# slp-rl/slamkit

Measured on NVIDIA H100. Metric: speech-tokens/sec (SLAM seq=1024), higher is better.
Workload: dtype bf16

## Files before the change

slamkit_b200/csrc/common.cuh:

```cuda
#pragma once
#include <cuda_runtime.h>
#include <cuda_bf16.h>
#include <cuda.h>
#include <stdint.h>
#include <stdio.h>

#define SK_DEVINL __device__ __forceinline__

typedef __nv_bfloat16 bf16;
typedef __nv_bfloat162 bf162;

void sk_set_error(const char* fmt, ...);
#define SK_CUDA_CHECK(expr)                                                            \
  do {                                                                                 \
    cudaError_t _e = (expr);                                                           \
    if (_e != cudaSuccess) {                                                           \
      sk_set_error("%s:%d: %s -> %s", __FILE__, __LINE__, #expr, cudaGetErrorString(_e)); \
      return -2;                                                                       \
    }                                                                                  \
  } while (0)
void sk_count_launch();
#define SK_LAUNCH_CHECK()            \
  do {                               \
    sk_count_launch();               \
    SK_CUDA_CHECK(cudaGetLastError()); \
  } while (0)
#define SK_REQUIRE(cond, ...)                  \
  do {                                         \
    if (!(cond)) {                             \
      sk_set_error(__VA_ARGS__);               \
      return -1;                               \
    }                                          \
  } while (0)

int sk_num_sms();

#ifdef __CUDACC__
__device__ __forceinline__ void griddep_wait() { asm volatile("griddepcontrol.wait;" ::: "memory"); }
__device__ __forceinline__ void griddep_launch() { asm volatile("griddepcontrol.launch_dependents;" ::: "memory"); }
#endif
bool sk_pdl_enabled();
template <typename... KArgs, typename... Args>
inline cudaError_t sk_launch_pdl_if(bool pdl, void (*kernel)(KArgs...), dim3 grid, dim3 block, size_t smem, cudaStream_t s,
                                    Args... args) {
  cudaLaunchConfig_t cfg = {};
  cfg.gridDim = grid;
  cfg.blockDim = block;
  cfg.dynamicSmemBytes = smem;
  cfg.stream = s;
  cudaLaunchAttribute attr[1];
  attr[0].id = cudaLaunchAttributeProgrammaticStreamSerialization;
  attr[0].val.programmaticStreamSerializationAllowed = 1;
  cfg.attrs = attr;
  cfg.numAttrs = (pdl && sk_pdl_enabled()) ? 1 : 0;
  return cudaLaunchKernelEx(&cfg, kernel, static_cast<KArgs>(args)...);
}
template <typename... KArgs, typename... Args>
inline cudaError_t sk_launch_pdl(void (*kernel)(KArgs...), dim3 grid, dim3 block, size_t smem, cudaStream_t s, Args... args) {
  return sk_launch_pdl_if(true, kernel, grid, block, smem, s, args...);
}
void sk_prof_begin(int cat, cudaStream_t s);
void sk_prof_end(cudaStream_t s);

SK_DEVINL uint32_t pack_bf16(float lo, float hi) {
  bf162 v = __floats2bfloat162_rn(lo, hi);
  return *reinterpret_cast<uint32_t*>(&v);
}
SK_DEVINL float2 unpack_bf16(uint32_t v) {
  bf162 b = *reinterpret_cast<bf162*>(&v);
  return __bfloat1622float2(b);
}
SK_DEVINL float bf16_round(float x) { return __bfloat162float(__float2bfloat16_rn(x)); }

SK_DEVINL float warp_sum(float v) {
#pragma unroll
  for (int o = 16; o > 0; o >>= 1) v += __shfl_xor_sync(0xffffffffu, v, o);
  return v;
}
SK_DEVINL float warp_max(float v) {
#pragma unroll
  for (int o = 16; o > 0; o >>= 1) v = fmaxf(v, __shfl_xor_sync(0xffffffffu, v, o));
  return v;
}

SK_DEVINL uint4 ldg128(const void* p) { return __ldg(reinterpret_cast<const uint4*>(p)); }
SK_DEVINL uint4 ldg128_stream(const void* p) {
  uint4 r;
  asm volatile("ld.global.nc.L1::no_allocate.v4.u32 {%0,%1,%2,%3}, [%4];"
               : "=r"(r.x), "=r"(r.y), "=r"(r.z), "=r"(r.w)
               : "l"(p));
  return r;
}
SK_DEVINL void stg128(void* p, uint4 v) { *reinterpret_cast<uint4*>(p) = v; }

SK_DEVINL uint32_t smem_u32(const void* p) { return static_cast<uint32_t>(__cvta_generic_to_shared(p)); }

SK_DEVINL uint32_t elect_one() {
  uint32_t pred = 0;
  asm volatile(
      "{\n\t.reg .pred P;\n\t"
      "elect.sync _|P, 0xffffffff;\n\t"
      "selp.u32 %0, 1, 0, P;\n\t}\n"
      : "=r"(pred));
  return pred;
}

SK_DEVINL void mbar_init(uint32_t bar, uint32_t count) {
  asm volatile("mbarrier.init.shared::cta.b64 [%0], %1;" ::"r"(bar), "r"(count) : "memory");
}
SK_DEVINL void fence_mbar_init() { asm volatile("fence.mbarrier_init.release.cluster;" ::: "memory"); }
SK_DEVINL void fence_proxy_async() { asm volatile("fence.proxy.async.shared::cta;" ::: "memory"); }
SK_DEVINL void mbar_arrive(uint32_t bar) {
  asm volatile("mbarrier.arrive.shared::cta.b64 _, [%0];" ::"r"(bar) : "memory");
}
SK_DEVINL void mbar_arrive_expect_tx(uint32_t bar, uint32_t bytes) {
  asm volatile("mbarrier.arrive.expect_tx.shared::cta.b64 _, [%0], %1;" ::"r"(bar), "r"(bytes) : "memory");
}
SK_DEVINL uint32_t mbar_try_wait(uint32_t bar, uint32_t parity) {
  uint32_t ok;
  asm volatile(
      "{\n\t.reg .pred P;\n\t"
      "mbarrier.try_wait.parity.shared::cta.b64 P, [%1], %2;\n\t"
      "selp.u32 %0, 1, 0, P;\n\t}\n"
      : "=r"(ok)
      : "r"(bar), "r"(parity)
      : "memory");
  return ok;
}
SK_DEVINL uint64_t globaltimer_ns() {
  uint64_t t;
  asm volatile("mov.u64 %0, %%globaltimer;" : "=l"(t));
  return t;
}
SK_DEVINL float ex2_approx(float x) {
  float y;
  asm("ex2.approx.ftz.f32 %0, %1;" : "=f"(y) : "f"(x));
  return y;
}

SK_DEVINL float sigmoid_f(float x) {
  float r;
  asm("rcp.approx.ftz.f32 %0, %1;" : "=f"(r) : "f"(1.0f + ex2_approx(x * -1.4426950408889634f)));
  return r;
}
SK_DEVINL float silu_f(float x) { return x * sigmoid_f(x); }

typedef float2 f32x2;
SK_DEVINL f32x2 pk2(float a, float b) { return make_float2(a, b); }
SK_DEVINL void upk2(f32x2 v, float& a, float& b) { a = v.x; b = v.y; }
SK_DEVINL f32x2 dup2(float c) { return make_float2(c, c); }
SK_DEVINL f32x2 fma2(f32x2 a, f32x2 b, f32x2 c) { return make_float2(__fmaf_rn(a.x, b.x, c.x), __fmaf_rn(a.y, b.y, c.y)); }
SK_DEVINL f32x2 mul2(f32x2 a, f32x2 b) { return make_float2(__fmul_rn(a.x, b.x), __fmul_rn(a.y, b.y)); }
SK_DEVINL f32x2 add2(f32x2 a, f32x2 b) { return make_float2(__fadd_rn(a.x, b.x), __fadd_rn(a.y, b.y)); }
SK_DEVINL f32x2 sub2(f32x2 a, f32x2 b) { return make_float2(__fsub_rn(a.x, b.x), __fsub_rn(a.y, b.y)); }
SK_DEVINL void mbar_wait_sleep(uint32_t bar, uint32_t parity) {
  if (mbar_try_wait(bar, parity)) return;
  uint64_t t0 = globaltimer_ns();
  uint32_t spins = 0;
  while (!mbar_try_wait(bar, parity)) {
    __nanosleep(40);
    if ((++spins & 0xfffu) == 0 && globaltimer_ns() - t0 > 4000000000ull) {
      printf("slamkit_b200: mbarrier wait timeout (block %d thread %d bar 0x%x parity %u)\n", blockIdx.x, threadIdx.x, bar,
             parity);
      __trap();
    }
  }
}
SK_DEVINL void mbar_wait(uint32_t bar, uint32_t parity) {
  if (mbar_try_wait(bar, parity)) return;
  uint64_t t0 = globaltimer_ns();
  uint32_t spins = 0;
  while (!mbar_try_wait(bar, parity)) {
    if ((++spins & 0x3fffu) == 0) {
      if (globaltimer_ns() - t0 > 4000000000ull) {
        printf("slamkit_b200: mbarrier wait timeout (block %d thread %d bar 0x%x parity %u)\n", blockIdx.x,
               threadIdx.x, bar, parity);
        __trap();
      }
    }
  }
}

SK_DEVINL void mbar_wait_nocall(uint32_t bar, uint32_t parity) {
  if (mbar_try_wait(bar, parity)) return;
  uint64_t t0 = globaltimer_ns();
  uint32_t spins = 0;
  while (!mbar_try_wait(bar, parity)) {
    if ((++spins & 0x3fffu) == 0 && globaltimer_ns() - t0 > 4000000000ull) __trap();
  }
}

SK_DEVINL void tma_prefetch_desc(const void* tmap) {
  asm volatile("prefetch.tensormap [%0];" ::"l"(tmap) : "memory");
}
SK_DEVINL void tma_load_2d(uint32_t smem_dst, const void* tmap, uint32_t bar, int32_t c0, int32_t c1) {
  asm volatile(
      "cp.async.bulk.tensor.2d.shared::cluster.global.mbarrier::complete_tx::bytes [%0], [%1, {%3, %4}], [%2];"
      ::"r"(smem_dst), "l"(tmap), "r"(bar), "r"(c0), "r"(c1)
      : "memory");
}
SK_DEVINL void tma_load_3d(uint32_t smem_dst, const void* tmap, uint32_t bar, int32_t c0, int32_t c1, int32_t c2) {
  asm volatile(
      "cp.async.bulk.tensor.3d.shared::cluster.global.mbarrier::complete_tx::bytes [%0], [%1, {%3, %4, %5}], [%2];"
      ::"r"(smem_dst), "l"(tmap), "r"(bar), "r"(c0), "r"(c1), "r"(c2)
      : "memory");
}
SK_DEVINL void tma_store_2d(const void* tmap, uint32_t smem_src, int32_t c0, int32_t c1) {
  asm volatile("cp.async.bulk.tensor.2d.global.shared::cta.bulk_group [%0, {%2, %3}], [%1];" ::"l"(tmap),
               "r"(smem_src), "r"(c0), "r"(c1)
               : "memory");
}
SK_DEVINL void tma_store_commit() { asm volatile("cp.async.bulk.commit_group;" ::: "memory"); }
template <int N>
SK_DEVINL void tma_store_wait_read() {
  asm volatile("cp.async.bulk.wait_group.read %0;" ::"n"(N) : "memory");
}
template <int N>
SK_DEVINL void tma_store_wait() {
  asm volatile("cp.async.bulk.wait_group %0;" ::"n"(N) : "memory");
}

SK_DEVINL void wgmma_fence() { asm volatile("wgmma.fence.sync.aligned;" ::: "memory"); }
SK_DEVINL void wgmma_commit() { asm volatile("wgmma.commit_group.sync.aligned;" ::: "memory"); }
template <int N>
SK_DEVINL void wgmma_wait() {
  asm volatile("wgmma.wait_group.sync.aligned %0;" ::"n"(N) : "memory");
}
SK_DEVINL void named_bar_sync(int id, int threads) { asm volatile("bar.sync %0, %1;" ::"r"(id), "r"(threads) : "memory"); }

SK_DEVINL uint64_t gmma_desc_sw128(uint32_t smem_addr, uint32_t lbo_bytes, uint32_t sbo_bytes) {
  uint64_t d = 0;
  d |= (uint64_t)((smem_addr & 0x3ffffu) >> 4);
  d |= (uint64_t)((lbo_bytes >> 4) & 0x3fffu) << 16;
  d |= (uint64_t)((sbo_bytes >> 4) & 0x3fffu) << 32;
  d |= (uint64_t)1 << 62;
  return d;
}
template <int TA, int TB>
SK_DEVINL void wgmma_m64n64(float (&d)[32], uint64_t da, uint64_t db) {
  asm volatile(
      "{\n\t.reg .pred p;\n\tsetp.eq.u32 p, 1, 1;\n\t"
      "wgmma.mma_async.sync.aligned.m64n64k16.f32.bf16.bf16 {%0,%1,%2,%3,%4,%5,%6,%7,%8,%9,%10,%11,%12,%13,%14,%15,%16,%17,%18,%19,%20,%21,%22,%23,%24,%25,%26,%27,%28,%29,%30,%31}, %32, %33, p, 1, 1, %34, %35;\n\t}\n"
      : "+f"(d[0]), "+f"(d[1]), "+f"(d[2]), "+f"(d[3]), "+f"(d[4]), "+f"(d[5]), "+f"(d[6]), "+f"(d[7]), "+f"(d[8]), "+f"(d[9]), "+f"(d[10]), "+f"(d[11]), "+f"(d[12]), "+f"(d[13]), "+f"(d[14]), "+f"(d[15]), "+f"(d[16]), "+f"(d[17]), "+f"(d[18]), "+f"(d[19]), "+f"(d[20]), "+f"(d[21]), "+f"(d[22]), "+f"(d[23]), "+f"(d[24]), "+f"(d[25]), "+f"(d[26]), "+f"(d[27]), "+f"(d[28]), "+f"(d[29]), "+f"(d[30]), "+f"(d[31])
      : "l"(da), "l"(db), "n"(TA), "n"(TB));
}
template <int TA, int TB>
SK_DEVINL void wgmma_m64n128(float (&d)[64], uint64_t da, uint64_t db) {
  asm volatile(
      "{\n\t.reg .pred p;\n\tsetp.eq.u32 p, 1, 1;\n\t"
      "wgmma.mma_async.sync.aligned.m64n128k16.f32.bf16.bf16 {%0,%1,%2,%3,%4,%5,%6,%7,%8,%9,%10,%11,%12,%13,%14,%15,%16,%17,%18,%19,%20,%21,%22,%23,%24,%25,%26,%27,%28,%29,%30,%31,%32,%33,%34,%35,%36,%37,%38,%39,%40,%41,%42,%43,%44,%45,%46,%47,%48,%49,%50,%51,%52,%53,%54,%55,%56,%57,%58,%59,%60,%61,%62,%63}, %64, %65, p, 1, 1, %66, %67;\n\t}\n"
      : "+f"(d[0]), "+f"(d[1]), "+f"(d[2]), "+f"(d[3]), "+f"(d[4]), "+f"(d[5]), "+f"(d[6]), "+f"(d[7]), "+f"(d[8]), "+f"(d[9]), "+f"(d[10]), "+f"(d[11]), "+f"(d[12]), "+f"(d[13]), "+f"(d[14]), "+f"(d[15]), "+f"(d[16]), "+f"(d[17]), "+f"(d[18]), "+f"(d[19]), "+f"(d[20]), "+f"(d[21]), "+f"(d[22]), "+f"(d[23]), "+f"(d[24]), "+f"(d[25]), "+f"(d[26]), "+f"(d[27]), "+f"(d[28]), "+f"(d[29]), "+f"(d[30]), "+f"(d[31]), "+f"(d[32]), "+f"(d[33]), "+f"(d[34]), "+f"(d[35]), "+f"(d[36]), "+f"(d[37]), "+f"(d[38]), "+f"(d[39]), "+f"(d[40]), "+f"(d[41]), "+f"(d[42]), "+f"(d[43]), "+f"(d[44]), "+f"(d[45]), "+f"(d[46]), "+f"(d[47]), "+f"(d[48]), "+f"(d[49]), "+f"(d[50]), "+f"(d[51]), "+f"(d[52]), "+f"(d[53]), "+f"(d[54]), "+f"(d[55]), "+f"(d[56]), "+f"(d[57]), "+f"(d[58]), "+f"(d[59]), "+f"(d[60]), "+f"(d[61]), "+f"(d[62]), "+f"(d[63])
      : "l"(da), "l"(db), "n"(TA), "n"(TB));
}
template <int TA, int TB>
SK_DEVINL void wgmma_m64n256(float (&d)[128], uint64_t da, uint64_t db) {
  asm volatile(
      "{\n\t.reg .pred p;\n\tsetp.eq.u32 p, 1, 1;\n\t"
      "wgmma.mma_async.sync.aligned.m64n256k16.f32.bf16.bf16 {%0,%1,%2,%3,%4,%5,%6,%7,%8,%9,%10,%11,%12,%13,%14,%15,%16,%17,%18,%19,%20,%21,%22,%23,%24,%25,%26,%27,%28,%29,%30,%31,%32,%33,%34,%35,%36,%37,%38,%39,%40,%41,%42,%43,%44,%45,%46,%47,%48,%49,%50,%51,%52,%53,%54,%55,%56,%57,%58,%59,%60,%61,%62,%63,%64,%65,%66,%67,%68,%69,%70,%71,%72,%73,%74,%75,%76,%77,%78,%79,%80,%81,%82,%83,%84,%85,%86,%87,%88,%89,%90,%91,%92,%93,%94,%95,%96,%97,%98,%99,%100,%101,%102,%103,%104,%105,%106,%107,%108,%109,%110,%111,%112,%113,%114,%115,%116,%117,%118,%119,%120,%121,%122,%123,%124,%125,%126,%127}, %128, %129, p, 1, 1, %130, %131;\n\t}\n"
      : "+f"(d[0]), "+f"(d[1]), "+f"(d[2]), "+f"(d[3]), "+f"(d[4]), "+f"(d[5]), "+f"(d[6]), "+f"(d[7]), "+f"(d[8]), "+f"(d[9]), "+f"(d[10]), "+f"(d[11]), "+f"(d[12]), "+f"(d[13]), "+f"(d[14]), "+f"(d[15]), "+f"(d[16]), "+f"(d[17]), "+f"(d[18]), "+f"(d[19]), "+f"(d[20]), "+f"(d[21]), "+f"(d[22]), "+f"(d[23]), "+f"(d[24]), "+f"(d[25]), "+f"(d[26]), "+f"(d[27]), "+f"(d[28]), "+f"(d[29]), "+f"(d[30]), "+f"(d[31]), "+f"(d[32]), "+f"(d[33]), "+f"(d[34]), "+f"(d[35]), "+f"(d[36]), "+f"(d[37]), "+f"(d[38]), "+f"(d[39]), "+f"(d[40]), "+f"(d[41]), "+f"(d[42]), "+f"(d[43]), "+f"(d[44]), "+f"(d[45]), "+f"(d[46]), "+f"(d[47]), "+f"(d[48]), "+f"(d[49]), "+f"(d[50]), "+f"(d[51]), "+f"(d[52]), "+f"(d[53]), "+f"(d[54]), "+f"(d[55]), "+f"(d[56]), "+f"(d[57]), "+f"(d[58]), "+f"(d[59]), "+f"(d[60]), "+f"(d[61]), "+f"(d[62]), "+f"(d[63]), "+f"(d[64]), "+f"(d[65]), "+f"(d[66]), "+f"(d[67]), "+f"(d[68]), "+f"(d[69]), "+f"(d[70]), "+f"(d[71]), "+f"(d[72]), "+f"(d[73]), "+f"(d[74]), "+f"(d[75]), "+f"(d[76]), "+f"(d[77]), "+f"(d[78]), "+f"(d[79]), "+f"(d[80]), "+f"(d[81]), "+f"(d[82]), "+f"(d[83]), "+f"(d[84]), "+f"(d[85]), "+f"(d[86]), "+f"(d[87]), "+f"(d[88]), "+f"(d[89]), "+f"(d[90]), "+f"(d[91]), "+f"(d[92]), "+f"(d[93]), "+f"(d[94]), "+f"(d[95]), "+f"(d[96]), "+f"(d[97]), "+f"(d[98]), "+f"(d[99]), "+f"(d[100]), "+f"(d[101]), "+f"(d[102]), "+f"(d[103]), "+f"(d[104]), "+f"(d[105]), "+f"(d[106]), "+f"(d[107]), "+f"(d[108]), "+f"(d[109]), "+f"(d[110]), "+f"(d[111]), "+f"(d[112]), "+f"(d[113]), "+f"(d[114]), "+f"(d[115]), "+f"(d[116]), "+f"(d[117]), "+f"(d[118]), "+f"(d[119]), "+f"(d[120]), "+f"(d[121]), "+f"(d[122]), "+f"(d[123]), "+f"(d[124]), "+f"(d[125]), "+f"(d[126]), "+f"(d[127])
      : "l"(da), "l"(db), "n"(TA), "n"(TB));
}
template <int N, int TA, int TB>
SK_DEVINL void wgmma_bf16(float (&d)[N / 2], uint64_t da, uint64_t db) {
  if constexpr (N == 256) wgmma_m64n256<TA, TB>(d, da, db);
  else if constexpr (N == 128) wgmma_m64n128<TA, TB>(d, da, db);
  else wgmma_m64n64<TA, TB>(d, da, db);
}
```

slamkit_b200/csrc/gemm_tcgen05.cu:

```cuda
#include "common.cuh"
#include <cudaTypedefs.h>
#include <stdio.h>
#include <mutex>
#include <string.h>
#include <stdlib.h>
#include "kernels.h"
#include "../../include/slamkit_b200.h"

namespace {

constexpr int BM = 128;
constexpr int BK = 64;
constexpr int MMA_K = 16;
constexpr int GEMM_THREADS = 288;


struct GemmParams {
  int M, N, K;
  int batch;
  int a_mode;
  int passes;
  void* C;
  void* C_lo;
  int ldc;
  const void* bias;
  int bias_f32;
  const bf16* residual;
  const bf16* residual_lo;
  int ldr;
  int tiles_m, tiles_n;
  int out_f32;
  int round_before_res;
  int act;
  int col_gin, col_gout;
  int splits;
  float* splitk_ws;
  int tma_store;
  int pdl;
  int sk_units;
  int sk_groups;
  int sk_G;
  int sk_colunits;
  int units, n_groups;
  float* sk_ws;
  uint32_t* sk_flags;
  int epi;
  const bf16* aux;
  int ld_aux;
  const bf16* rope_cos;
  const bf16* rope_sin;
  const int* rope_pos;
  int rope_T, rope_cols, rope_maxpos;
};

template <int BN, int EW = 4>
struct GemmCfg {
  static constexpr int A_BYTES = BM * BK * 2;
  static constexpr int B_ATOMS = (BN + 63) / 64;
  static constexpr int B_BYTES = B_ATOMS * 64 * BK * 2;
  static constexpr int STAGE_BYTES = A_BYTES + B_BYTES;
  static constexpr int STAGES = (BN > 128) ? 4 : (BN > 64 ? 6 : 8);
  static constexpr int STAGING_BYTES = 4 * 2 * 4096;
  static constexpr int BAR_BYTES = 256;
  static constexpr int SMEM_BYTES = STAGES * STAGE_BYTES + STAGING_BYTES + BAR_BYTES + 1024;
  static_assert(STAGES * STAGE_BYTES >= BM * BN * 4, "the parked fp32 accumulator must fit in the stage ring");
  static_assert(SMEM_BYTES <= 227 * 1024, "sm_90 allows 227 KB of shared memory per block");
};

template <int BN>
SK_DEVINL uint32_t acc_chunk_addr(uint32_t base, int row, int chunk) {
  return base + (uint32_t)row * (BN * 4) + (uint32_t)((chunk ^ (row & 7)) << 4);
}
template <int BN>
SK_DEVINL void acc_park(uint32_t base, const float (&d)[BN / 2], int wg, int warp_in_wg, int lane) {
  const int r0 = 64 * wg + 16 * warp_in_wg + (lane >> 2);
#pragma unroll
  for (int j = 0; j < BN / 8; ++j) {
    const int chunk = 2 * j + ((lane & 3) >> 1);
    const uint32_t off = (uint32_t)(lane & 1) * 8u;
    asm volatile("st.shared.v2.f32 [%0], {%1, %2};" ::"r"(acc_chunk_addr<BN>(base, r0, chunk) + off), "f"(d[4 * j]),
                 "f"(d[4 * j + 1]) : "memory");
    asm volatile("st.shared.v2.f32 [%0], {%1, %2};" ::"r"(acc_chunk_addr<BN>(base, r0 + 8, chunk) + off), "f"(d[4 * j + 2]),
                 "f"(d[4 * j + 3]) : "memory");
  }
}
template <int BN>
SK_DEVINL void acc_ld_32x32(uint32_t base, uint32_t ta, uint32_t (&r)[32]) {
  const int row = (int)(ta >> 16) + (int)(threadIdx.x & 31);
  const int c0 = (int)(ta & 0xffffu) >> 2;
#pragma unroll
  for (int i = 0; i < 8; ++i)
    asm volatile("ld.shared.v4.b32 {%0, %1, %2, %3}, [%4];"
                 : "=r"(r[4 * i]), "=r"(r[4 * i + 1]), "=r"(r[4 * i + 2]), "=r"(r[4 * i + 3])
                 : "r"(acc_chunk_addr<BN>(base, row, c0 + i)) : "memory");
}

SK_DEVINL float gelu_erf(float y) {
  const float a = fabsf(y);
  float t;
  asm("rcp.approx.ftz.f32 %0, %1;" : "=f"(t) : "f"(fmaf(0.3275911f * 0.70710678118654752440f, a, 1.0f)));
  float s = fmaf(0.5f * 1.061405429f, t, 0.5f * -1.453152027f);
  s = fmaf(s, t, 0.5f * 1.421413741f);
  s = fmaf(s, t, 0.5f * -0.284496736f);
  s = fmaf(s, t, 0.5f * 0.254829592f);
  const float e = ex2_approx((y * y) * -0.72134752044448170368f);
  return fmaf(-a, (s * t) * e, fmaxf(y, 0.0f));
}

template <bool SK>
struct WorkIter {
  int num_kb, splits, kb_per_split, total_items, tiles_n;
  int G, colunits, units, n_groups, sk_groups, grp, mem;
  long sk_total, sk_cur, sk_end;
  int next_unit, next_item;
  int tile, split, kb_begin, kb_end, role;
  long unit_end_it;
  SK_DEVINL WorkIter(const GemmParams& p, int num_kb_, int kb_per_split_, int total_items_) {
    num_kb = num_kb_;
    splits = p.splits;
    kb_per_split = kb_per_split_;
    total_items = total_items_;
    tiles_n = p.tiles_n;
    G = p.sk_G;
    colunits = p.sk_colunits;
    units = p.units;
    n_groups = p.n_groups;
    sk_groups = p.sk_groups;
    tile = split = kb_begin = kb_end = role = 0;
    unit_end_it = 0;
    sk_total = sk_cur = sk_end = 0;
    next_item = (int)blockIdx.x;
    next_unit = 0;
    grp = mem = 0;
    if (SK && p.sk_units > 0) {
      grp = (int)blockIdx.x / G;
      mem = (int)blockIdx.x - grp * G;
      next_item = total_items;
      next_unit = grp < n_groups ? p.sk_units + grp : units;
      if (grp < sk_groups) {
        sk_total = (long)p.sk_units * num_kb;
        sk_cur = sk_total * grp / sk_groups;
        sk_end = sk_total * (grp + 1) / sk_groups;
      }
    }
  }
  SK_DEVINL int tile_of(int unit) const { return colunits ? mem * tiles_n + unit : unit * G + mem; }
  SK_DEVINL bool next() {
    if (SK && sk_cur < sk_end) {
      const int unit = (int)(sk_cur / num_kb);
      kb_begin = (int)(sk_cur - (long)unit * num_kb);
      unit_end_it = (long)(unit + 1) * num_kb;
      const long e = sk_end < unit_end_it ? sk_end : unit_end_it;
      kb_end = kb_begin + (int)(e - sk_cur);
      tile = tile_of(unit);
      split = 0;
      role = kb_begin != 0 ? 1 : (e < unit_end_it ? 2 : 0);
      sk_cur = e;
      return true;
    }
    if (SK && next_unit < units) {
      tile = tile_of(next_unit);
      split = 0;
      kb_begin = 0;
      kb_end = num_kb;
      role = 0;
      next_unit += n_groups;
      return true;
    }
    if (next_item < total_items) {
      split = next_item % splits;
      tile = next_item / splits;
      kb_begin = split * kb_per_split;
      kb_end = min(num_kb, kb_begin + kb_per_split);
      role = 0;
      next_item += (int)gridDim.x;
      return true;
    }
    return false;
  }
  SK_DEVINL int n_contrib() const {
    int n = 0;
    for (int g = grp + 1; g < sk_groups && sk_total * g / sk_groups < unit_end_it; ++g) ++n;
    return n;
  }
};

SK_DEVINL uint32_t ld_acquire_u32(const uint32_t* p) {
  uint32_t v;
  asm volatile("ld.acquire.gpu.global.u32 %0, [%1];" : "=r"(v) : "l"(p) : "memory");
  return v;
}
SK_DEVINL void st_release_u32(uint32_t* p, uint32_t v) {
  asm volatile("st.release.gpu.global.u32 [%0], %1;" ::"l"(p), "r"(v) : "memory");
}

SK_DEVINL void epi_bias_act(float (&v)[8], const GemmParams& p, int col) {
  if (p.bias) {
    if (p.bias_f32) {
      const float* bp = reinterpret_cast<const float*>(p.bias) + col;
      const float4 b0 = __ldg(reinterpret_cast<const float4*>(bp));
      const float4 b1 = __ldg(reinterpret_cast<const float4*>(bp + 4));
      v[0] += b0.x; v[1] += b0.y; v[2] += b0.z; v[3] += b0.w;
      v[4] += b1.x; v[5] += b1.y; v[6] += b1.z; v[7] += b1.w;
    } else {
      const uint4 bv = ldg128(reinterpret_cast<const bf16*>(p.bias) + col);
      const uint32_t bw[4] = {bv.x, bv.y, bv.z, bv.w};
#pragma unroll
      for (int i = 0; i < 4; ++i) {
        const float2 f = unpack_bf16(bw[i]);
        v[2 * i] += f.x;
        v[2 * i + 1] += f.y;
      }
    }
  }
  if (p.act == 1) {
#pragma unroll
    for (int i = 0; i < 8; ++i) v[i] = gelu_erf(v[i]);
  } else if (p.act == 2) {
#pragma unroll
    for (int i = 0; i < 8; ++i) v[i] = fmaxf(v[i], 0.0f);
  }
}

SK_DEVINL void epi_residual(float (&v)[8], const GemmParams& p, size_t row, int ocol) {
  if (!p.residual) return;
  const uint4 rv = *reinterpret_cast<const uint4*>(p.residual + row * p.ldr + ocol);
  const uint32_t rw[4] = {rv.x, rv.y, rv.z, rv.w};
#pragma unroll
  for (int i = 0; i < 4; ++i) {
    const float2 f = unpack_bf16(rw[i]);
    if (p.round_before_res) {
      v[2 * i] = bf16_round(v[2 * i]) + f.x;
      v[2 * i + 1] = bf16_round(v[2 * i + 1]) + f.y;
    } else {
      v[2 * i] += f.x;
      v[2 * i + 1] += f.y;
    }
  }
  if (p.residual_lo) {
    const uint4 lv = *reinterpret_cast<const uint4*>(p.residual_lo + row * p.ldr + ocol);
    const uint32_t lw[4] = {lv.x, lv.y, lv.z, lv.w};
#pragma unroll
    for (int i = 0; i < 4; ++i) {
      const float2 f = unpack_bf16(lw[i]);
      v[2 * i] += f.x;
      v[2 * i + 1] += f.y;
    }
  }
}

constexpr int SK_SLOT_FLOATS = BM * 256;
SK_DEVINL size_t sk_slot_off(int chunk, int j4, int row_in_tile) { return ((size_t)(chunk * 8 + j4) * BM + row_in_tile) * 4; }

SK_DEVINL void sk_fixup_add(uint32_t (&r)[32], const float* ws, int chunk, int row_in_tile, int first_cta, int G, int n) {
  for (int c0 = 0; c0 < n; ++c0) {
    const float* slot = ws + (size_t)(first_cta + c0 * G) * SK_SLOT_FLOATS;
    float4 a[8];
#pragma unroll
    for (int j = 0; j < 8; ++j) a[j] = __ldcg(reinterpret_cast<const float4*>(slot + sk_slot_off(chunk, j, row_in_tile)));
#pragma unroll
    for (int j = 0; j < 8; ++j) {
      r[4 * j + 0] = __float_as_uint(__uint_as_float(r[4 * j + 0]) + a[j].x);
      r[4 * j + 1] = __float_as_uint(__uint_as_float(r[4 * j + 1]) + a[j].y);
      r[4 * j + 2] = __float_as_uint(__uint_as_float(r[4 * j + 2]) + a[j].z);
      r[4 * j + 3] = __float_as_uint(__uint_as_float(r[4 * j + 3]) + a[j].w);
    }
  }
}

template <int BN, bool A_MN, bool B_MN, bool SK, int EW>
__global__ void __launch_bounds__(GEMM_THREADS, 1)
gemm_wgmma_kernel(const __grid_constant__ CUtensorMap tmA, const __grid_constant__ CUtensorMap tmB,
                  const __grid_constant__ CUtensorMap tmA_lo, const __grid_constant__ CUtensorMap tmB_lo,
                  const __grid_constant__ CUtensorMap tmC, const __grid_constant__ CUtensorMap tmAux, GemmParams p) {
  using Cfg = GemmCfg<BN, EW>;
  static_assert(EW == 4 || (EW == 8 && BN == 256 && !SK), "8 epilogue warps: plain 256-wide tiles only");
  constexpr int CS = EW / 4;
  griddep_launch();
  extern __shared__ uint8_t smem_raw[];
  const uint32_t smem_base = (smem_u32(smem_raw) + 1023u) & ~1023u;
  const uint32_t staging_base = smem_base + Cfg::STAGES * Cfg::STAGE_BYTES;
  const uint32_t bar_base = staging_base + Cfg::STAGING_BYTES;
  auto full_bar = [&](int s) { return bar_base + 8u * s; };
  auto empty_bar = [&](int s) { return bar_base + 8u * (Cfg::STAGES + s); };
  const uint32_t acc_free = bar_base + 8u * (2 * Cfg::STAGES);

  const int warp = threadIdx.x >> 5;
  const int lane = threadIdx.x & 31;
  const int tiles_per_batch = p.tiles_m * p.tiles_n;
  const int total_items = tiles_per_batch * p.batch * p.splits;
  const int num_kb_total = (p.K + BK - 1) / BK;
  const int kb_per_split = (num_kb_total + p.splits - 1) / p.splits;
  constexpr uint32_t STAGE_TX = Cfg::A_BYTES + (B_MN ? Cfg::B_ATOMS * 64 * BK * 2 : BN * BK * 2);

  if (threadIdx.x == 0) {
    tma_prefetch_desc(&tmA);
    tma_prefetch_desc(&tmB);
    for (int s = 0; s < Cfg::STAGES; ++s) {
      mbar_init(full_bar(s), 1);
      mbar_init(empty_bar(s), 8);
    }
    mbar_init(acc_free, 1);
    fence_mbar_init();
  }
  __syncthreads();
  griddep_wait();

  if (warp == 8) {
    if (lane == 0) {
      const bool split = p.passes == 3;
      const int n_stage = split ? Cfg::STAGES / 2 : Cfg::STAGES;
      const uint32_t stage_bytes = split ? 2u * Cfg::STAGE_BYTES : (uint32_t)Cfg::STAGE_BYTES;
      int stage = 0;
      uint32_t phase = 0;
      uint32_t acc_phase = 0;
      bool first = true;
      WorkIter<SK> w(p, num_kb_total, kb_per_split, total_items);
      while (w.next()) {
        if (!first) {
          mbar_wait_nocall(acc_free, acc_phase);
          acc_phase ^= 1u;
        }
        first = false;
        const int bidx = w.tile / tiles_per_batch;
        const int r = w.tile - bidx * tiles_per_batch;
        const int m0 = (r / p.tiles_n) * BM;
        const int n_blk = r % p.tiles_n;
        const int n0 = n_blk * BN;
        for (int kb = w.kb_begin; kb < w.kb_end; ++kb) {
          mbar_wait_nocall(empty_bar(stage), phase ^ 1u);
          const uint32_t fb = full_bar(stage);
          mbar_arrive_expect_tx(fb, split ? 2u * STAGE_TX : STAGE_TX);
          for (int part = 0; part < (split ? 2 : 1); ++part) {
            const CUtensorMap* mapA = part ? &tmA_lo : &tmA;
            const CUtensorMap* mapB = part ? &tmB_lo : &tmB;
            const uint32_t sA = smem_base + stage * stage_bytes + part * Cfg::STAGE_BYTES;
            const uint32_t sB = sA + Cfg::A_BYTES;
            if (!A_MN) {
              if (p.a_mode & 2) {
                if (p.a_mode & 1) tma_load_3d(sA, mapA, fb, n_blk * 64, m0 + kb, bidx);
                else tma_load_3d(sA, mapA, fb, kb * BK, m0, bidx);
              } else {
                tma_load_2d(sA, mapA, fb, kb * BK, m0);
              }
            } else {
#pragma unroll
              for (int j = 0; j < BM / 64; ++j) tma_load_2d(sA + j * (BK * 128), mapA, fb, m0 + 64 * j, kb * BK);
            }
            if (!B_MN) {
              tma_load_2d(sB, mapB, fb, kb * BK, n0);
            } else {
#pragma unroll
              for (int j = 0; j < Cfg::B_ATOMS; ++j) tma_load_2d(sB + j * (BK * 128), mapB, fb, n0 + 64 * j, kb * BK);
            }
          }
          if (++stage == n_stage) { stage = 0; phase ^= 1u; }
        }
      }
    }
  } else {
    const int wg = warp >> 2;
    const int q = warp & 3;
    const int chalf = warp >> 2;
    const bool epi_warp = warp < EW;
    auto acc_ld = [&](uint32_t ta, uint32_t (&r)[32]) { acc_ld_32x32<BN>(smem_base, ta, r); };
    const bool split = p.passes == 3;
    const int n_stage = split ? Cfg::STAGES / 2 : Cfg::STAGES;
    const uint32_t stage_bytes = split ? 2u * Cfg::STAGE_BYTES : (uint32_t)Cfg::STAGE_BYTES;
    int stage = 0;
    uint32_t phase = 0;
    uint32_t store_cnt = 0;
    auto release_acc = [&] {
      fence_proxy_async();
      named_bar_sync(1, 256);
      if (threadIdx.x == 0) mbar_arrive(acc_free);
    };
    WorkIter<SK> w(p, num_kb_total, kb_per_split, total_items);
    while (w.next()) {
      {
        float acc[BN / 2];
#pragma unroll
        for (int i = 0; i < BN / 2; ++i) acc[i] = 0.f;
        const int k_iters = max(0, w.kb_end - w.kb_begin);
        int prev = -1;
        for (int kb = 0; kb < k_iters; ++kb) {
          mbar_wait_nocall(full_bar(stage), phase);
          wgmma_fence();
          const uint32_t s_hi = smem_base + stage * stage_bytes;
          for (int g = 0; g < (split ? 3 : 1); ++g) {
            const uint32_t sA = s_hi + (g == 2 ? Cfg::STAGE_BYTES : 0) + (uint32_t)wg * 8192u;
            const uint32_t sB = s_hi + Cfg::A_BYTES + (g == 1 ? Cfg::STAGE_BYTES : 0);
#pragma unroll
            for (int k = 0; k < BK / MMA_K; ++k) {
              const uint64_t adesc = A_MN ? gmma_desc_sw128(sA + k * (MMA_K * 128), BK * 128, 1024)
                                          : gmma_desc_sw128(sA + k * (MMA_K * 2), 16, 1024);
              const uint64_t bdesc = B_MN ? gmma_desc_sw128(sB + k * (MMA_K * 128), BK * 128, 1024)
                                          : gmma_desc_sw128(sB + k * (MMA_K * 2), 16, 1024);
              wgmma_bf16<BN, A_MN ? 1 : 0, B_MN ? 1 : 0>(acc, adesc, bdesc);
            }
          }
          wgmma_commit();
          wgmma_wait<1>();
          if (prev >= 0 && lane == 0) mbar_arrive(empty_bar(prev));
          prev = stage;
          if (++stage == n_stage) { stage = 0; phase ^= 1u; }
        }
        wgmma_wait<0>();
        if (prev >= 0 && lane == 0) mbar_arrive(empty_bar(prev));
        named_bar_sync(1, 256);
        acc_park<BN>(smem_base, acc, wg, warp & 3, lane);
        named_bar_sync(1, 256);
      }
      if (!epi_warp) {
        release_acc();
        continue;
      }
      const int split_idx = w.split;
      const int bidx = w.tile / tiles_per_batch;
      const int rr = w.tile - bidx * tiles_per_batch;
      const int m0 = (rr / p.tiles_n) * BM;
      const int n0 = (rr % p.tiles_n) * BN;
      if (!SK && p.tma_store && p.epi == 2) {
        const int lpiece = lane & 7, lrsub = lane >> 3;
        const uint32_t sX = staging_base + (uint32_t)warp * (EW == 4 ? 8192u : 4096u);
        constexpr int NCH = BN / 64 / CS;
        const int c_lo = chalf * NCH;
        auto piece_off = [&](int bidx, int m0, int n0, int c2, size_t ld) -> size_t {
          const int acol = n0 + c2 * 64;
          const int gcol = (acol >> 7) * 256 + (acol & 127) + lpiece * 8;
          return (((size_t)bidx * p.M + m0 + q * 32 + lrsub) * ld + gcol) * sizeof(bf16);
        };
        const size_t row4_in = (size_t)4 * p.ld_aux * sizeof(bf16), row4_out = (size_t)4 * p.ldc * sizeof(bf16);
        uint4 gv[8], uv[8];
        auto gu_load_k = [&](int k, const uint8_t* base, int m0, int n0, int c2) {
          const int rin = m0 + q * 32 + 4 * k + lrsub;
          if (rin < p.M && n0 + c2 * 64 < p.N) {
            gv[k] = ldg128(base + k * row4_in);
            uv[k] = ldg128(base + k * row4_in + 256);
          } else {
            gv[k] = make_uint4(0u, 0u, 0u, 0u);
            uv[k] = make_uint4(0u, 0u, 0u, 0u);
          }
        };
        {
          const uint8_t* base = reinterpret_cast<const uint8_t*>(p.aux) + piece_off(bidx, m0, n0, c_lo, (size_t)p.ld_aux);
#pragma unroll
          for (int k = 0; k < 8; ++k) gu_load_k(k, base, m0, n0, c_lo);
        }
        const uint32_t taddr = (uint32_t)(q * 32) << 16;
#pragma unroll 1
        for (int c2 = c_lo; c2 < c_lo + NCH; ++c2) {
          const bool col_ok = n0 + c2 * 64 < p.N;
          {
            uint32_t r0[32], r1[32];
            acc_ld(taddr + c2 * 64, r0);
            acc_ld(taddr + c2 * 64 + 32, r1);
#pragma unroll
            for (int j = 0; j < 8; ++j) {
              const uint32_t* r = j < 4 ? r0 + 8 * j : r1 + 8 * (j - 4);
              const uint32_t dst = sX + (uint32_t)lane * 128u + (uint32_t)((j ^ (lane & 7)) << 4);
              asm volatile("st.shared.v4.b32 [%0], {%1, %2, %3, %4};" ::"r"(dst),
                           "r"(pack_bf16(__uint_as_float(r[0]), __uint_as_float(r[1]))),
                           "r"(pack_bf16(__uint_as_float(r[2]), __uint_as_float(r[3]))),
                           "r"(pack_bf16(__uint_as_float(r[4]), __uint_as_float(r[5]))),
                           "r"(pack_bf16(__uint_as_float(r[6]), __uint_as_float(r[7])))
                           : "memory");
            }
          }
          __syncwarp();
          const bool refill = c2 + 1 < c_lo + NCH;
          const int fm0 = m0, fn0 = n0, fc2 = c2 + 1;
          const uint8_t* fbase = reinterpret_cast<const uint8_t*>(p.aux) + piece_off(bidx, fm0, fn0, fc2, (size_t)p.ld_aux);
          uint8_t* obase = reinterpret_cast<uint8_t*>(p.C) + piece_off(bidx, m0, n0, c2, (size_t)p.ldc);
#pragma unroll
          for (int k = 0; k < 8; ++k) {
            const int rr2 = 4 * k + lrsub;
            const uint32_t off = (uint32_t)rr2 * 128u + (uint32_t)((lpiece ^ (rr2 & 7)) << 4);
            uint32_t dw[4];
            asm volatile("ld.shared.v4.b32 {%0, %1, %2, %3}, [%4];" : "=r"(dw[0]), "=r"(dw[1]), "=r"(dw[2]), "=r"(dw[3]) : "r"(sX + off));
            const uint32_t gw[4] = {gv[k].x, gv[k].y, gv[k].z, gv[k].w}, uw[4] = {uv[k].x, uv[k].y, uv[k].z, uv[k].w};
            if (refill) gu_load_k(k, fbase, fm0, fn0, fc2);
            uint32_t og[4], ou[4];
#pragma unroll
            for (int e = 0; e < 4; ++e) {
              const float2 gf = unpack_bf16(gw[e]);
              const float s0 = sigmoid_f(gf.x), s1 = sigmoid_f(gf.y);
              const uint32_t sil2 = pack_bf16(gf.x * s0, gf.y * s1);
              const float ds0 = s0 * (1.0f + gf.x * (1.0f - s0)), ds1 = s1 * (1.0f + gf.y * (1.0f - s1));
              const bf162 d2 = *reinterpret_cast<const bf162*>(&dw[e]);
              bf162 du2 = __hmul2(d2, *reinterpret_cast<const bf162*>(&uw[e]));
              bf162 o2 = __hmul2(d2, *reinterpret_cast<const bf162*>(&sil2));
              const float2 duf = __bfloat1622float2(du2);
              og[e] = pack_bf16(duf.x * ds0, duf.y * ds1);
              ou[e] = *reinterpret_cast<uint32_t*>(&o2);
            }
            if (col_ok && m0 + q * 32 + rr2 < p.M) {
              stg128(obase + k * row4_out, make_uint4(og[0], og[1], og[2], og[3]));
              stg128(obase + k * row4_out + 256, make_uint4(ou[0], ou[1], ou[2], ou[3]));
            }
          }
          __syncwarp();
        }
        release_acc();
        continue;
      }
      const int row_in_tile = q * 32 + lane;
      const int row_in = m0 + row_in_tile;
      const bool row_ok = row_in < p.M;
      const size_t row = (size_t)bidx * p.M + row_in;
      const uint32_t taddr = (uint32_t)(q * 32) << 16;
      const int first_contrib = (int)blockIdx.x + w.G;
      const int n_contrib = (SK && w.role == 2) ? w.n_contrib() : 0;
      if (SK && w.role == 1) {
        float* slot = p.sk_ws + (size_t)blockIdx.x * SK_SLOT_FLOATS;
#pragma unroll 1
        for (int c = 0; c < BN / 32; ++c) {
          uint32_t r[32];
          acc_ld(taddr + c * 32, r);
#pragma unroll
          for (int j = 0; j < 8; ++j)
            __stcg(reinterpret_cast<float4*>(slot + sk_slot_off(c, j, row_in_tile)),
                   make_float4(__uint_as_float(r[4 * j]), __uint_as_float(r[4 * j + 1]), __uint_as_float(r[4 * j + 2]),
                               __uint_as_float(r[4 * j + 3])));
        }
        __threadfence();
        __syncwarp();
        if (lane == 0) st_release_u32(p.sk_flags + blockIdx.x * 4 + q, 1u);
      } else {
        if (SK && w.role == 2) {
          if (lane == 0) {
            for (int i = 0; i < n_contrib; ++i) {
              const int c = first_contrib + i * w.G;
              const uint32_t* f = p.sk_flags + c * 4 + q;
              const uint64_t t0 = globaltimer_ns();
              while (ld_acquire_u32(f) == 0u) {
                __nanosleep(64);
                if (globaltimer_ns() - t0 > 8000000000ull) __trap();
              }
            }
          }
          __syncwarp();
        }
        auto stage_store = [&](const CUtensorMap* map, const uint32_t (&pk)[32], int col) {
          const uint32_t sbuf = staging_base + (EW == 4 ? (uint32_t)warp * 8192u + (store_cnt & 1u) * 4096u : (uint32_t)warp * 4096u);
          if (lane == 0) {
            if constexpr (EW == 4) tma_store_wait_read<1>(); else tma_store_wait_read<0>();
          }
          __syncwarp();
#pragma unroll
          for (int j = 0; j < 8; ++j) {
            const uint32_t dst = sbuf + (uint32_t)lane * 128u + (uint32_t)((j ^ (lane & 7)) << 4);
            asm volatile("st.shared.v4.b32 [%0], {%1, %2, %3, %4};" ::"r"(dst), "r"(pk[4 * j]), "r"(pk[4 * j + 1]),
                         "r"(pk[4 * j + 2]), "r"(pk[4 * j + 3])
                         : "memory");
          }
          fence_proxy_async();
          __syncwarp();
          if (lane == 0) {
            tma_store_2d(map, sbuf, col, m0 + q * 32);
            tma_store_commit();
          }
          ++store_cnt;
        };
        if (!SK && p.tma_store && p.epi == 1) {
          if constexpr (BN == 256) {
#pragma unroll 1
#pragma unroll 1
            for (int i = chalf * (2 / CS); i < (chalf + 1) * (2 / CS); ++i) {
              uint32_t gpk[32], upk[32];
              {
                uint32_t r0[32], r1[32];
                acc_ld(taddr + i * 64, r0);
                acc_ld(taddr + i * 64 + 32, r1);
#pragma unroll
                for (int t = 0; t < 16; ++t) {
                  gpk[t] = pack_bf16(__uint_as_float(r0[2 * t]), __uint_as_float(r0[2 * t + 1]));
                  gpk[16 + t] = pack_bf16(__uint_as_float(r1[2 * t]), __uint_as_float(r1[2 * t + 1]));
                }
              }
              stage_store(&tmC, gpk, n0 + i * 64);
              {
                uint32_t r0[32], r1[32];
                acc_ld(taddr + 128 + i * 64, r0);
                acc_ld(taddr + 128 + i * 64 + 32, r1);
#pragma unroll
                for (int t = 0; t < 16; ++t) {
                  upk[t] = pack_bf16(__uint_as_float(r0[2 * t]), __uint_as_float(r0[2 * t + 1]));
                  upk[16 + t] = pack_bf16(__uint_as_float(r1[2 * t]), __uint_as_float(r1[2 * t + 1]));
                }
              }
              stage_store(&tmC, upk, n0 + 128 + i * 64);
#pragma unroll
              for (int t = 0; t < 32; ++t) {
                const float2 gf = unpack_bf16(gpk[t]), uf = unpack_bf16(upk[t]);
                const float2 sb = unpack_bf16(pack_bf16(silu_f(gf.x), silu_f(gf.y)));
                gpk[t] = pack_bf16(sb.x * uf.x, sb.y * uf.y);
              }
              stage_store(&tmAux, gpk, (n0 >> 1) + i * 64);
            }
          }
        } else if (!SK && p.tma_store && p.epi == 3) {
          uint32_t cw[16], sw[16];
          {
            int pos = 0;
            if (row_ok) pos = p.rope_pos ? p.rope_pos[row] : (int)(row % (size_t)p.rope_T);
            pos = max(0, min(pos, p.rope_maxpos - 1));
#pragma unroll
            for (int j = 0; j < 4; ++j) {
              const uint4 c = ldg128(p.rope_cos + (size_t)pos * 32 + 8 * j), sn = ldg128(p.rope_sin + (size_t)pos * 32 + 8 * j);
              cw[4 * j] = c.x; cw[4 * j + 1] = c.y; cw[4 * j + 2] = c.z; cw[4 * j + 3] = c.w;
              sw[4 * j] = sn.x; sw[4 * j + 1] = sn.y; sw[4 * j + 2] = sn.z; sw[4 * j + 3] = sn.w;
            }
          }
#pragma unroll 1
          for (int c2 = chalf * (BN / 64 / CS); c2 < (chalf + 1) * (BN / 64 / CS); ++c2) {
            const int col64 = n0 + c2 * 64;
            if (col64 >= p.N) break;
            uint32_t r0[32], r1[32], pk[32];
            acc_ld(taddr + c2 * 64, r0);
            acc_ld(taddr + c2 * 64 + 32, r1);
#pragma unroll
            for (int g = 0; g < 4; ++g) {
              float v0[8], v1[8];
#pragma unroll
              for (int i = 0; i < 8; ++i) {
                v0[i] = __uint_as_float(r0[g * 8 + i]);
                v1[i] = __uint_as_float(r1[g * 8 + i]);
              }
              if (p.bias) {
                const uint4 b0 = ldg128(reinterpret_cast<const bf16*>(p.bias) + col64 + g * 8);
                const uint4 b1 = ldg128(reinterpret_cast<const bf16*>(p.bias) + col64 + 32 + g * 8);
                const uint32_t w0[4] = {b0.x, b0.y, b0.z, b0.w}, w1[4] = {b1.x, b1.y, b1.z, b1.w};
#pragma unroll
                for (int e = 0; e < 4; ++e) {
                  const float2 f0 = unpack_bf16(w0[e]), f1 = unpack_bf16(w1[e]);
                  v0[2 * e] += f0.x; v0[2 * e + 1] += f0.y;
                  v1[2 * e] += f1.x; v1[2 * e + 1] += f1.y;
                }
              }
              if (col64 < p.rope_cols) {
#pragma unroll
                for (int e = 0; e < 4; ++e) {
                  const float2 c = unpack_bf16(cw[g * 4 + e]), sn = unpack_bf16(sw[g * 4 + e]);
                  const float2 x1 = unpack_bf16(pack_bf16(v0[2 * e], v0[2 * e + 1]));
                  const float2 x2 = unpack_bf16(pack_bf16(v1[2 * e], v1[2 * e + 1]));
                  v0[2 * e] = bf16_round(x1.x * c.x) + bf16_round(-x2.x * sn.x);
                  v0[2 * e + 1] = bf16_round(x1.y * c.y) + bf16_round(-x2.y * sn.y);
                  v1[2 * e] = bf16_round(x2.x * c.x) + bf16_round(x1.x * sn.x);
                  v1[2 * e + 1] = bf16_round(x2.y * c.y) + bf16_round(x1.y * sn.y);
                }
              }
#pragma unroll
              for (int e = 0; e < 4; ++e) {
                pk[g * 4 + e] = pack_bf16(v0[2 * e], v0[2 * e + 1]);
                pk[16 + g * 4 + e] = pack_bf16(v1[2 * e], v1[2 * e + 1]);
              }
            }
            stage_store(&tmC, pk, col64);
          }
        } else if (p.tma_store && !p.bias && !p.residual && !p.act) {
#pragma unroll 1
          for (int c2 = chalf * (BN / 64 / CS); c2 < (chalf + 1) * (BN / 64 / CS); ++c2) {
            uint32_t r0[32], r1[32], pk[32];
            acc_ld(taddr + c2 * 64, r0);
            acc_ld(taddr + c2 * 64 + 32, r1);
            if (SK && n_contrib > 0) {
              sk_fixup_add(r0, p.sk_ws, c2 * 2, row_in_tile, first_contrib, w.G, n_contrib);
              sk_fixup_add(r1, p.sk_ws, c2 * 2 + 1, row_in_tile, first_contrib, w.G, n_contrib);
            }
#pragma unroll
            for (int t = 0; t < 16; ++t) {
              pk[t] = pack_bf16(__uint_as_float(r0[2 * t]), __uint_as_float(r0[2 * t + 1]));
              pk[16 + t] = pack_bf16(__uint_as_float(r1[2 * t]), __uint_as_float(r1[2 * t + 1]));
            }
            stage_store(&tmC, pk, n0 + c2 * 64);
          }
        } else if (p.tma_store && !p.bias && !p.act && p.residual && !p.residual_lo) {
#pragma unroll 1
          for (int c2 = chalf * (BN / 64 / CS); c2 < (chalf + 1) * (BN / 64 / CS); ++c2) {
            const int col64 = n0 + c2 * 64;
            if (col64 >= p.N) break;
            uint4 rv[8];
            if (row_ok) {
              const bf16* rp = p.residual + row * p.ldr + col64;
#pragma unroll
              for (int j = 0; j < 8; ++j) rv[j] = (col64 + 8 * j < p.N) ? ldg128(rp + 8 * j) : make_uint4(0u, 0u, 0u, 0u);
            } else {
#pragma unroll
              for (int j = 0; j < 8; ++j) rv[j] = make_uint4(0u, 0u, 0u, 0u);
            }
            uint32_t r0[32], r1[32], pk[32];
            acc_ld(taddr + c2 * 64, r0);
            acc_ld(taddr + c2 * 64 + 32, r1);
            if (SK && n_contrib > 0) {
              sk_fixup_add(r0, p.sk_ws, c2 * 2, row_in_tile, first_contrib, w.G, n_contrib);
              sk_fixup_add(r1, p.sk_ws, c2 * 2 + 1, row_in_tile, first_contrib, w.G, n_contrib);
            }
#pragma unroll
            for (int j = 0; j < 8; ++j) {
              const uint32_t* r = j < 4 ? r0 + 8 * j : r1 + 8 * (j - 4);
              const uint32_t rw[4] = {rv[j].x, rv[j].y, rv[j].z, rv[j].w};
#pragma unroll
              for (int e = 0; e < 4; ++e) {
                const float2 f = unpack_bf16(rw[e]);
                float a0 = __uint_as_float(r[2 * e]), a1 = __uint_as_float(r[2 * e + 1]);
                if (p.round_before_res) {
                  const float2 t = unpack_bf16(pack_bf16(a0, a1));
                  a0 = t.x; a1 = t.y;
                }
                pk[4 * j + e] = pack_bf16(a0 + f.x, a1 + f.y);
              }
            }
            stage_store(&tmC, pk, col64);
          }
        } else if (p.tma_store) {
#pragma unroll 1
          for (int c2 = chalf * (BN / 64 / CS); c2 < (chalf + 1) * (BN / 64 / CS); ++c2) {
            const uint32_t sbuf = staging_base + (EW == 4 ? (uint32_t)warp * 8192u + (store_cnt & 1u) * 4096u : (uint32_t)warp * 4096u);
            if (lane == 0) {
              if constexpr (EW == 4) tma_store_wait_read<1>(); else tma_store_wait_read<0>();
            }
            __syncwarp();
#pragma unroll
            for (int half = 0; half < 2; ++half) {
              uint32_t r[32];
              acc_ld(taddr + c2 * 64 + half * 32, r);
              if (SK && n_contrib > 0) sk_fixup_add(r, p.sk_ws, c2 * 2 + half, row_in_tile, first_contrib, w.G, n_contrib);
#pragma unroll
              for (int g = 0; g < 4; ++g) {
                const int col = n0 + c2 * 64 + half * 32 + g * 8;
                float v[8];
#pragma unroll
                for (int i = 0; i < 8; ++i) v[i] = __uint_as_float(r[g * 8 + i]);
                if (col < p.N) {
                  epi_bias_act(v, p, col);
                  if (row_ok) epi_residual(v, p, row, col);
                }
                const int j = half * 4 + g;
                const uint32_t dst = sbuf + (uint32_t)lane * 128u + (uint32_t)((j ^ (lane & 7)) << 4);
                asm volatile("st.shared.v4.b32 [%0], {%1, %2, %3, %4};" ::"r"(dst), "r"(pack_bf16(v[0], v[1])),
                             "r"(pack_bf16(v[2], v[3])), "r"(pack_bf16(v[4], v[5])), "r"(pack_bf16(v[6], v[7]))
                             : "memory");
              }
            }
            fence_proxy_async();
            __syncwarp();
            if (lane == 0) {
              tma_store_2d(&tmC, sbuf, n0 + c2 * 64, m0 + q * 32);
              tma_store_commit();
            }
            ++store_cnt;
          }
        }
        else
#pragma unroll 1
        for (int c = chalf * (BN / 32 / CS); c < (chalf + 1) * (BN / 32 / CS); ++c) {
          uint32_t r[32];
          acc_ld(taddr + c * 32, r);
          if (SK && n_contrib > 0) sk_fixup_add(r, p.sk_ws, c, row_in_tile, first_contrib, w.G, n_contrib);
          const int col0 = n0 + c * 32;
          if (row_ok && col0 < p.N) {
#pragma unroll
            for (int g = 0; g < 4; ++g) {
              const int col = col0 + g * 8;
              if (col < p.N) {
                float v[8];
#pragma unroll
                for (int i = 0; i < 8; ++i) v[i] = __uint_as_float(r[g * 8 + i]);
                if (p.splits > 1) {
                  float* dst = p.splitk_ws + ((size_t)split_idx * p.M + row_in) * p.N + col;
                  *reinterpret_cast<float4*>(dst) = make_float4(v[0], v[1], v[2], v[3]);
                  *reinterpret_cast<float4*>(dst + 4) = make_float4(v[4], v[5], v[6], v[7]);
                  continue;
                }
                epi_bias_act(v, p, col);
                int ocol = col;
                if (p.col_gin > 0) {
                  const int gi = col / p.col_gin, ci = col - gi * p.col_gin;
                  if (ci >= p.col_gout) continue;
                  ocol = gi * p.col_gout + ci;
                }
                epi_residual(v, p, row, ocol);
                if (p.out_f32) {
                  float* dst = reinterpret_cast<float*>(p.C) + row * p.ldc + ocol;
                  *reinterpret_cast<float4*>(dst) = make_float4(v[0], v[1], v[2], v[3]);
                  *reinterpret_cast<float4*>(dst + 4) = make_float4(v[4], v[5], v[6], v[7]);
                } else {
                  uint4 o;
                  o.x = pack_bf16(v[0], v[1]);
                  o.y = pack_bf16(v[2], v[3]);
                  o.z = pack_bf16(v[4], v[5]);
                  o.w = pack_bf16(v[6], v[7]);
                  stg128(reinterpret_cast<bf16*>(p.C) + row * p.ldc + ocol, o);
                  if (p.C_lo) {
                    const float2 h0 = unpack_bf16(o.x), h1 = unpack_bf16(o.y), h2 = unpack_bf16(o.z), h3 = unpack_bf16(o.w);
                    uint4 l;
                    l.x = pack_bf16(v[0] - h0.x, v[1] - h0.y);
                    l.y = pack_bf16(v[2] - h1.x, v[3] - h1.y);
                    l.z = pack_bf16(v[4] - h2.x, v[5] - h2.y);
                    l.w = pack_bf16(v[6] - h3.x, v[7] - h3.y);
                    stg128(reinterpret_cast<bf16*>(p.C_lo) + row * p.ldc + ocol, l);
                  }
                }
              }
            }
          }
        }
        if (SK && w.role == 2) {
          __syncwarp();
          if (lane == 0)
            for (int i = 0; i < n_contrib; ++i) p.sk_flags[(first_contrib + i * w.G) * 4 + q] = 0u;
        }
      }
      release_acc();
    }
    if (epi_warp && p.tma_store && lane == 0) tma_store_wait<0>();
  }
}

__global__ void splitk_reduce_kernel(const float* __restrict__ ws, bf16* __restrict__ C, int M, int N, int ldc, int splits,
                                     int accumulate, int round_before_res) {
  griddep_launch();
  griddep_wait();
  const long total = (long)M * N / 8;
  for (long i = blockIdx.x * (long)blockDim.x + threadIdx.x; i < total; i += (long)gridDim.x * blockDim.x) {
    const long e = i * 8;
    const int m = (int)(e / N), n = (int)(e % N);
    float acc[8] = {0, 0, 0, 0, 0, 0, 0, 0};
    for (int s = 0; s < splits; ++s) {
      const float* src = ws + ((size_t)s * M + m) * N + n;
      const float4 a = *reinterpret_cast<const float4*>(src), b = *reinterpret_cast<const float4*>(src + 4);
      acc[0] += a.x; acc[1] += a.y; acc[2] += a.z; acc[3] += a.w;
      acc[4] += b.x; acc[5] += b.y; acc[6] += b.z; acc[7] += b.w;
    }
    bf16* dst = C + (size_t)m * ldc + n;
    if (accumulate) {
      const uint4 o = *reinterpret_cast<const uint4*>(dst);
      const uint32_t ow[4] = {o.x, o.y, o.z, o.w};
#pragma unroll
      for (int k = 0; k < 4; ++k) {
        const float2 f = unpack_bf16(ow[k]);
        acc[2 * k] = (round_before_res ? bf16_round(acc[2 * k]) : acc[2 * k]) + f.x;
        acc[2 * k + 1] = (round_before_res ? bf16_round(acc[2 * k + 1]) : acc[2 * k + 1]) + f.y;
      }
    }
    stg128(dst, make_uint4(pack_bf16(acc[0], acc[1]), pack_bf16(acc[2], acc[3]), pack_bf16(acc[4], acc[5]),
                           pack_bf16(acc[6], acc[7])));
  }
}

PFN_cuTensorMapEncodeTiled_v12000 g_encode = nullptr;
std::once_flag g_encode_once;

void load_encode() {
  void* fn = nullptr;
  cudaDriverEntryPointQueryResult qres;
  cudaError_t e = cudaGetDriverEntryPoint("cuTensorMapEncodeTiled", &fn, cudaEnableDefault, &qres);
  if (e == cudaSuccess && qres == cudaDriverEntryPointSuccess) g_encode = (PFN_cuTensorMapEncodeTiled_v12000)fn;
}

}

int sk_make_tmap_2d(CUtensorMap* out, const void* ptr, int elem_bytes, uint64_t inner, uint64_t outer, uint64_t ld,
                    uint32_t box_inner, uint32_t box_outer) {
  std::call_once(g_encode_once, load_encode);
  SK_REQUIRE(g_encode != nullptr, "cuTensorMapEncodeTiled driver entry point not available");
  SK_REQUIRE((reinterpret_cast<uintptr_t>(ptr) & 15) == 0, "TMA base pointer must be 16-byte aligned");
  SK_REQUIRE((ld * elem_bytes) % 16 == 0, "TMA row pitch must be a multiple of 16 bytes (ld=%llu)",
             (unsigned long long)ld);
  SK_REQUIRE(box_inner * elem_bytes == 128, "SW128 box inner extent must be 128 bytes");
  cuuint64_t dims[2] = {inner, outer};
  cuuint64_t strides[1] = {ld * (uint64_t)elem_bytes};
  cuuint32_t box[2] = {box_inner, box_outer};
  cuuint32_t estr[2] = {1, 1};
  CUtensorMapDataType dt = elem_bytes == 2 ? CU_TENSOR_MAP_DATA_TYPE_BFLOAT16 : CU_TENSOR_MAP_DATA_TYPE_FLOAT32;
  CUresult r = g_encode(out, dt, 2, const_cast<void*>(ptr), dims, strides, box, estr, CU_TENSOR_MAP_INTERLEAVE_NONE,
                        CU_TENSOR_MAP_SWIZZLE_128B, CU_TENSOR_MAP_L2_PROMOTION_L2_256B,
                        CU_TENSOR_MAP_FLOAT_OOB_FILL_NONE);
  SK_REQUIRE(r == CUDA_SUCCESS, "cuTensorMapEncodeTiled failed with CUresult %d (inner=%llu outer=%llu ld=%llu)", (int)r,
             (unsigned long long)inner, (unsigned long long)outer, (unsigned long long)ld);
  return 0;
}

int sk_make_tmap_3d(CUtensorMap* out, const void* ptr, uint64_t inner, uint64_t rows, uint64_t batch, uint64_t row_stride,
                    uint64_t batch_stride, uint32_t box_rows) {
  std::call_once(g_encode_once, load_encode);
  SK_REQUIRE(g_encode != nullptr, "cuTensorMapEncodeTiled driver entry point not available");
  SK_REQUIRE((reinterpret_cast<uintptr_t>(ptr) & 15) == 0, "TMA base pointer must be 16-byte aligned");
  SK_REQUIRE((row_stride * 2) % 16 == 0 && (batch_stride * 2) % 16 == 0, "TMA strides must be multiples of 16 bytes");
  cuuint64_t dims[3] = {inner, rows, batch};
  cuuint64_t strides[2] = {row_stride * 2, batch_stride * 2};
  cuuint32_t box[3] = {64, box_rows, 1};
  cuuint32_t estr[3] = {1, 1, 1};
  CUresult r = g_encode(out, CU_TENSOR_MAP_DATA_TYPE_BFLOAT16, 3, const_cast<void*>(ptr), dims, strides, box, estr,
                        CU_TENSOR_MAP_INTERLEAVE_NONE, CU_TENSOR_MAP_SWIZZLE_128B, CU_TENSOR_MAP_L2_PROMOTION_L2_256B,
                        CU_TENSOR_MAP_FLOAT_OOB_FILL_NONE);
  SK_REQUIRE(r == CUDA_SUCCESS, "cuTensorMapEncodeTiled(3d) failed with CUresult %d", (int)r);
  return 0;
}

namespace {

template <int BN, bool A_MN, bool B_MN, bool SK, int EW = 4>
int launch_gemm(const CUtensorMap* tm, const GemmParams& p, int grid, cudaStream_t stream) {
  using Cfg = GemmCfg<BN, EW>;
  static bool attr_set = false;
  if (!attr_set) {
    SK_CUDA_CHECK(cudaFuncSetAttribute(gemm_wgmma_kernel<BN, A_MN, B_MN, SK, EW>, cudaFuncAttributeMaxDynamicSharedMemorySize,
                                       Cfg::SMEM_BYTES));
    attr_set = true;
  }
  sk_prof_begin(0, stream);
  cudaError_t lerr = sk_launch_pdl_if(p.pdl != 0, gemm_wgmma_kernel<BN, A_MN, B_MN, SK, EW>, dim3(grid), dim3(GEMM_THREADS), (size_t)Cfg::SMEM_BYTES, stream,
                                   tm[0], tm[1], tm[2], tm[3], tm[4], tm[5], p);
  sk_prof_end(stream);
  SK_CUDA_CHECK(lerr);
  SK_LAUNCH_CHECK();
  return 0;
}

template <int BN, bool SK, int EW = 4>
int dispatch_major(bool a_mn, bool b_mn, const CUtensorMap* tm, const GemmParams& p, int grid, cudaStream_t s) {
  if (!a_mn && !b_mn) return launch_gemm<BN, false, false, SK, EW>(tm, p, grid, s);
  if (!a_mn && b_mn) return launch_gemm<BN, false, true, SK, EW>(tm, p, grid, s);
  if (a_mn && !b_mn) return launch_gemm<BN, true, false, SK, EW>(tm, p, grid, s);
  return launch_gemm<BN, true, true, SK, EW>(tm, p, grid, s);
}

inline int tile_cost(int bn) { return bn >= 256 ? 100 : (bn >= 128 ? 61 : 54); }

constexpr size_t SK_FLAG_BYTES = 4096;

}

size_t sk_gemm_ws_min_bytes(void) { return (size_t)sk_num_sms() * SK_SLOT_FLOATS * sizeof(float) + SK_FLAG_BYTES; }

int sk_pick_bn(int M, int N, int force_bn) {
  if (force_bn == 64 || force_bn == 128 || force_bn == 256) return force_bn;
  const int nsm = sk_num_sms();
  const int cands[3] = {256, 128, 64};
  int best = 256;
  long best_cost = -1;
  for (int i = 0; i < 3; ++i) {
    const int bn = cands[i];
    const long tiles = (long)((M + BM - 1) / BM) * ((N + bn - 1) / bn);
    const long waves = (tiles + nsm - 1) / nsm;
    const long cost = waves * tile_cost(bn);
    if (best_cost < 0 || cost * 100 < best_cost * 75) {
      best_cost = cost;
      best = bn;
    }
  }
  return best;
}

namespace {

int plan_gemm(const SkGemmEx& g, GemmParams& p, int& BN, int& ew, int& grid) {
  SK_REQUIRE(g.M > 0 && g.N > 0 && g.K > 0 && g.batch >= 1, "gemm: empty problem M=%d N=%d K=%d batch=%d", g.M, g.N, g.K,
             g.batch);
  SK_REQUIRE(g.N % 8 == 0, "gemm: N must be a multiple of 8 (N=%d)", g.N);
  SK_REQUIRE(g.ldc % 8 == 0 && (g.residual == nullptr || g.ldr % 8 == 0), "gemm: ldc/ldr must be multiples of 8");
  SK_REQUIRE((reinterpret_cast<uintptr_t>(g.C) & 15) == 0, "gemm: C must be 16-byte aligned");
  SK_REQUIRE(((reinterpret_cast<uintptr_t>(g.A) | reinterpret_cast<uintptr_t>(g.B) | reinterpret_cast<uintptr_t>(g.A_lo) |
               reinterpret_cast<uintptr_t>(g.B_lo)) & 15) == 0,
             "gemm: A and B must be 16-byte aligned");
  SK_REQUIRE((reinterpret_cast<uintptr_t>(g.bias) & 15) == 0 && (reinterpret_cast<uintptr_t>(g.residual) & 15) == 0,
             "gemm: bias and residual must be 16-byte aligned");
  SK_REQUIRE(g.passes == 1 || (g.passes == 3 && g.A_lo && g.B_lo), "gemm: passes must be 1, or 3 with lo operands");
  SK_REQUIRE(g.act >= 0 && g.act <= 2, "gemm: act must be 0 (none), 1 (GELU) or 2 (ReLU), got %d", g.act);
  const bool use3d = g.a_rows > 0;
  SK_REQUIRE(!use3d || !g.a_mn, "gemm: a batched / windowed A operand must be K-major");
  SK_REQUIRE(g.a_mode == 0 || use3d, "gemm: a_mode 1 needs the 3-D A view");
  SK_REQUIRE(use3d || g.lda >= (g.a_mn ? g.M : g.K), "gemm: lda=%d is smaller than the %s of A", g.lda, g.a_mn ? "M" : "K");
  SK_REQUIRE(g.ldb >= (g.b_mn ? g.N : g.K), "gemm: ldb=%d is smaller than the %s of B", g.ldb, g.b_mn ? "N" : "K");
  if (g.col_gin == 0) {
    const int out_cols = g.epi == 2 ? 2 * g.N : g.N;
    SK_REQUIRE(g.ldc >= out_cols, "gemm: ldc=%d is smaller than the %d output columns", g.ldc, out_cols);
    SK_REQUIRE(g.residual == nullptr || g.ldr >= g.N, "gemm: ldr=%d is smaller than N=%d", g.ldr, g.N);
  }
  const int nsm = sk_num_sms();
  static const int sk_env = [] { const char* e = getenv("SK_STREAMK"); return e ? atoi(e) : 1; }();
  static const int sk_min_idle = [] { const char* e = getenv("SK_STREAMK_MIN_IDLE"); return e ? atoi(e) : 20; }();
  static const int sk_min_kb = [] { const char* e = getenv("SK_STREAMK_MIN_KB"); return e ? atoi(e) : 32; }();
  const bool sk_ok = sk_env != 0 && g.batch == 1 && !use3d && g.passes == 1 && g.a_mode == 0 && g.splitk_ws != nullptr &&
                     g.splitk_ws_bytes >= sk_gemm_ws_min_bytes();
  const size_t ws_data_bytes = g.splitk_ws_bytes > SK_FLAG_BYTES ? g.splitk_ws_bytes - SK_FLAG_BYTES : 0;
  BN = (g.a_mode == 1) ? 64 : sk_pick_bn(g.M * g.batch, g.N, (g.epi == 1 || g.epi == 2) ? 256 : g.force_bn);
  memset(&p, 0, sizeof(p));
  p.M = g.M; p.N = g.N; p.K = g.K;
  p.batch = g.batch;
  p.a_mode = (g.a_mode & 1) | (use3d ? 2 : 0);
  p.passes = g.passes;
  p.C = g.C; p.C_lo = g.C_lo; p.ldc = g.ldc;
  p.bias = g.bias; p.bias_f32 = g.bias_f32;
  p.residual = reinterpret_cast<const bf16*>(g.residual);
  p.residual_lo = reinterpret_cast<const bf16*>(g.residual_lo);
  p.ldr = g.ldr;
  p.tiles_m = (g.M + BM - 1) / BM;
  p.tiles_n = (g.N + BN - 1) / BN;
  p.out_f32 = g.out_f32;
  p.round_before_res = g.round_before_res;
  p.act = g.act;
  p.col_gin = g.col_gin; p.col_gout = g.col_gout;
  p.pdl = g.pdl;
  const long tiles = (long)p.tiles_m * p.tiles_n * g.batch;
  p.splits = 1;
  p.splitk_ws = nullptr;
  const int num_kb = (g.K + BK - 1) / BK;
  static const int splitk_env = [] { const char* e = getenv("SK_SPLITK"); return e ? atoi(e) : 1; }();
  static const int sk_ranges = [] { const char* e = getenv("SK_STREAMK_RANGES"); return e ? atoi(e) : 4; }();
  if (splitk_env && g.splitk_ws && g.batch == 1 && g.passes == 1 && !g.out_f32 && !g.bias && !g.act && !g.C_lo && g.col_gin == 0 &&
      (g.residual == nullptr || g.residual == g.C) && tiles * 2 <= nsm && num_kb >= 16) {
    int sp = (int)(nsm / tiles);
    if (sp > 8) sp = 8;
    if (sp > num_kb / 4) sp = num_kb / 4;
    if ((size_t)sp * g.M * g.N * sizeof(float) > ws_data_bytes) sp = (int)(ws_data_bytes / ((size_t)g.M * g.N * sizeof(float)));
    if (sp >= 2) {
      const int per = (num_kb + sp - 1) / sp;
      sp = (num_kb + per - 1) / per;
    }
    if (sp >= 2) {
      p.splits = sp;
      p.splitk_ws = reinterpret_cast<float*>(g.splitk_ws);
    }
  }
  p.tma_store = (!g.out_f32 && !g.C_lo && g.col_gin == 0 && p.splits == 1 && g.batch == 1 && !use3d && (g.ldc * 2) % 16 == 0)
                    ? 1 : 0;
  p.epi = g.epi;
  p.aux = reinterpret_cast<const bf16*>(g.aux);
  p.ld_aux = g.ld_aux;
  p.rope_cos = reinterpret_cast<const bf16*>(g.rope_cos);
  p.rope_sin = reinterpret_cast<const bf16*>(g.rope_sin);
  p.rope_pos = g.rope_pos;
  p.rope_T = g.rope_T; p.rope_cols = g.rope_cols; p.rope_maxpos = g.rope_maxpos;
  if (g.epi != 0) {
    SK_REQUIRE(p.tma_store && g.passes == 1 && !g.residual && !g.act && g.splitk_ws == nullptr,
               "gemm: fused epilogue %d needs the plain bf16 TMA-store path (no residual / activation / scratch)", g.epi);
    if (g.epi == 1) {
      SK_REQUIRE(BN == 256 && g.N % 256 == 0 && g.aux_out && g.ld_aux_out % 8 == 0 && !g.bias,
                 "gemm: SwiGLU-forward epilogue needs N = 2F with F %% 128 == 0 and an act output");
    } else if (g.epi == 2) {
      SK_REQUIRE(BN == 256 && g.N % 128 == 0 && g.aux && g.ld_aux % 8 == 0 && !g.bias,
                 "gemm: SwiGLU-backward epilogue needs N = F with F %% 128 == 0 and the saved gu activation");
    } else if (g.epi == 3) {
      SK_REQUIRE(g.rope_cos && g.rope_sin && g.rope_T > 0 && g.rope_maxpos > 0 && g.rope_cols % 64 == 0 && g.N % 64 == 0 &&
                     !g.bias_f32,
                 "gemm: RoPE epilogue needs cos/sin tables, 64-column heads and a bf16 bias");
    } else {
      SK_REQUIRE(false, "gemm: unknown fused epilogue %d", g.epi);
    }
  }
  p.sk_G = 1;
  if (sk_ok && BN == 256 && p.splits == 1 && num_kb >= sk_min_kb && (p.tiles_n <= 8 || (sk_env >= 2 && p.tiles_m <= 8))) {
    const int colunits = p.tiles_n <= 8 ? 0 : 1;
    const int G = colunits ? p.tiles_m : p.tiles_n;
    const int units = colunits ? p.tiles_n : p.tiles_m;
    const int n_groups = nsm / G;
    const int rem = units % n_groups;
    const long slots = ((long)(units + n_groups - 1) / n_groups) * n_groups;
    if (n_groups >= 1 && rem != 0 && (slots - units) * 100 >= slots * sk_min_idle) {
      p.sk_units = rem;
      p.sk_groups = n_groups < rem * sk_ranges ? n_groups : rem * sk_ranges;
      p.sk_G = G;
      p.sk_colunits = colunits;
      p.units = units;
      p.n_groups = n_groups;
      p.sk_ws = reinterpret_cast<float*>(g.splitk_ws);
      p.sk_flags = reinterpret_cast<uint32_t*>(reinterpret_cast<uint8_t*>(g.splitk_ws) + ws_data_bytes);
    }
  }
  const long work = tiles * p.splits;
  grid = p.sk_units > 0 ? p.n_groups * p.sk_G : (int)(work < nsm ? work : nsm);
  static const int ew_env = [] { const char* e = getenv("SK_GEMM_EW"); return e ? atoi(e) : 0; }();
  ew = (p.sk_units == 0 && BN == 256 && p.tma_store && (ew_env == 8 || (ew_env == 0 && (g.epi == 2 || g.epi == 3)))) ? 8 : 4;
  return 0;
}

}

int sk_gemm_plan_ex(const SkGemmEx& g, SkGemmPlan* out) {
  GemmParams p;
  int BN = 0, ew = 0, grid = 0;
  const int rc = plan_gemm(g, p, BN, ew, grid);
  if (rc) return rc;
  out->bn = BN;
  out->epi_warps = ew;
  out->splits = p.splits;
  out->sk_units = p.sk_units;
  out->sk_groups = p.sk_groups;
  out->sk_G = p.sk_G;
  out->sk_colunits = p.sk_colunits;
  out->tma_store = p.tma_store;
  out->grid = grid;
  return 0;
}

int sk_gemm_ex_launch(const SkGemmEx& g, cudaStream_t stream) {
  GemmParams p;
  int BN = 0, ew = 0, grid = 0;
  const int rc0 = plan_gemm(g, p, BN, ew, grid);
  if (rc0) return rc0;
  const bool use3d = g.a_rows > 0;
  CUtensorMap tm[6];
  const void* As[2] = {g.A, g.passes == 3 ? g.A_lo : g.A};
  const void* Bs[2] = {g.B, g.passes == 3 ? g.B_lo : g.B};
  for (int i = 0; i < 2; ++i) {
    int rc;
    CUtensorMap* ta = &tm[i == 0 ? 0 : 2];
    CUtensorMap* tb = &tm[i == 0 ? 1 : 3];
    if (use3d) {
      rc = sk_make_tmap_3d(ta, As[i], (uint64_t)g.a_inner, (uint64_t)g.a_rows, (uint64_t)g.batch, (uint64_t)g.a_row_stride,
                           (uint64_t)g.a_batch_stride, BM);
    } else if (!g.a_mn) {
      rc = sk_make_tmap_2d(ta, As[i], 2, (uint64_t)g.K, (uint64_t)g.M, (uint64_t)g.lda, BK, BM);
    } else {
      rc = sk_make_tmap_2d(ta, As[i], 2, (uint64_t)g.M, (uint64_t)g.K, (uint64_t)g.lda, 64, BK);
    }
    if (rc) return rc;
    if (!g.b_mn) rc = sk_make_tmap_2d(tb, Bs[i], 2, (uint64_t)g.K, (uint64_t)g.N, (uint64_t)g.ldb, BK, (uint32_t)BN);
    else         rc = sk_make_tmap_2d(tb, Bs[i], 2, (uint64_t)g.N, (uint64_t)g.K, (uint64_t)g.ldb, 64, BK);
    if (rc) return rc;
  }
  tm[4] = tm[0];
  if (p.tma_store) {
    const int rc2 = sk_make_tmap_2d(&tm[4], g.C, 2, (uint64_t)(g.epi == 2 ? 2 * g.N : g.N), (uint64_t)g.M, (uint64_t)g.ldc, 64, 32);
    if (rc2) return rc2;
  }
  tm[5] = tm[4];
  if (g.epi == 1) {
    const int rc3 = sk_make_tmap_2d(&tm[5], g.aux_out, 2, (uint64_t)g.N / 2, (uint64_t)g.M, (uint64_t)g.ld_aux_out, 64, 32);
    if (rc3) return rc3;
  }
  int rc;
  if (p.sk_units > 0) {
    rc = dispatch_major<256, true>(g.a_mn, g.b_mn, tm, p, grid, stream);
  } else if (ew == 8) {
    rc = dispatch_major<256, false, 8>(g.a_mn, g.b_mn, tm, p, grid, stream);
  } else {
    switch (BN) {
      case 256: rc = dispatch_major<256, false>(g.a_mn, g.b_mn, tm, p, grid, stream); break;
      case 128: rc = dispatch_major<128, false>(g.a_mn, g.b_mn, tm, p, grid, stream); break;
      default:  rc = dispatch_major<64, false>(g.a_mn, g.b_mn, tm, p, grid, stream); break;
    }
  }
  if (rc) return rc;
  if (p.splits > 1) {
    SK_REQUIRE(g.residual == nullptr || g.residual == g.C, "gemm: split-K supports only in-place accumulation");
    const long n8 = (long)g.M * g.N / 8;
    int blocks = (int)((n8 + 255) / 256);
    if (blocks > sk_num_sms() * 8) blocks = sk_num_sms() * 8;
    sk_prof_begin(0, stream);
    SK_CUDA_CHECK(sk_launch_pdl(splitk_reduce_kernel, dim3(blocks), dim3(256), (size_t)(0), stream, p.splitk_ws, reinterpret_cast<bf16*>(g.C), g.M, g.N, g.ldc, p.splits,
                                                     g.residual != nullptr, g.round_before_res));
    sk_prof_end(stream);
    SK_LAUNCH_CHECK();
  }
  return 0;
}

SkGemmEx sk_gemm_desc(int M, int N, int K, const void* A, int lda, int a_mn, const void* B, int ldb, int b_mn, void* C,
                      int ldc, int out_f32, const void* bias, const void* residual, int ldr, int round_before_res, int act,
                      int force_bn, void* splitk_ws, size_t splitk_ws_bytes) {
  SkGemmEx g;
  memset(&g, 0, sizeof(g));
  g.M = M; g.N = N; g.K = K; g.batch = 1; g.passes = 1;
  g.A = A; g.lda = lda; g.a_mn = a_mn;
  g.B = B; g.ldb = ldb; g.b_mn = b_mn;
  g.C = C; g.ldc = ldc; g.out_f32 = out_f32;
  g.bias = bias; g.residual = residual; g.ldr = ldr; g.round_before_res = round_before_res; g.act = act;
  g.force_bn = force_bn;
  g.pdl = 1;
  g.splitk_ws = splitk_ws;
  g.splitk_ws_bytes = splitk_ws_bytes;
  return g;
}
int sk_gemm_launch(int M, int N, int K, const void* A, int lda, int a_mn, const void* B, int ldb, int b_mn, void* C,
                   int ldc, int out_f32, const void* bias, const void* residual, int ldr, int round_before_res, int act,
                   int force_bn, cudaStream_t stream, void* splitk_ws, size_t splitk_ws_bytes) {
  return sk_gemm_ex_launch(sk_gemm_desc(M, N, K, A, lda, a_mn, B, ldb, b_mn, C, ldc, out_f32, bias, residual, ldr,
                                        round_before_res, act, force_bn, splitk_ws, splitk_ws_bytes),
                           stream);
}

int sk_linear_swiglu_fwd_launch(int M, int F, int K, const void* x, const void* Wgu, void* gu, void* act, cudaStream_t s) {
  SkGemmEx g;
  memset(&g, 0, sizeof(g));
  g.M = M; g.N = 2 * F; g.K = K; g.batch = 1; g.passes = 1;
  g.A = x; g.lda = K; g.B = Wgu; g.ldb = K;
  g.C = gu; g.ldc = 2 * F;
  g.epi = 1; g.aux_out = act; g.ld_aux_out = F;
  g.pdl = 1;
  return sk_gemm_ex_launch(g, s);
}
int sk_linear_swiglu_bwd_launch(int M, int N, int F, const void* dy, const void* Wd, const void* gu, void* dgu, cudaStream_t s) {
  SkGemmEx g;
  memset(&g, 0, sizeof(g));
  g.M = M; g.N = F; g.K = N; g.batch = 1; g.passes = 1;
  g.A = dy; g.lda = N; g.B = Wd; g.ldb = F; g.b_mn = 1;
  g.C = dgu; g.ldc = 2 * F;
  g.epi = 2; g.aux = gu; g.ld_aux = 2 * F;
  g.pdl = 1;
  return sk_gemm_ex_launch(g, s);
}
int sk_linear_rope_launch(int M, int N, int K, const void* x, const void* W, const void* bias, void* out, const void* cos_t,
                          const void* sin_t, const int32_t* pos_ids, int T, int rope_cols, int max_positions, cudaStream_t s) {
  SkGemmEx g;
  memset(&g, 0, sizeof(g));
  g.M = M; g.N = N; g.K = K; g.batch = 1; g.passes = 1;
  g.A = x; g.lda = K; g.B = W; g.ldb = K;
  g.C = out; g.ldc = N;
  g.bias = bias;
  g.epi = 3; g.rope_cos = cos_t; g.rope_sin = sin_t; g.rope_pos = pos_ids; g.rope_T = T;
  g.rope_cols = rope_cols; g.rope_maxpos = max_positions;
  g.pdl = 1;
  return sk_gemm_ex_launch(g, s);
}
```

slamkit_b200/csrc/kernels.h:

```cpp
#pragma once
#include "common.cuh"

int sk_make_tmap_2d(CUtensorMap* out, const void* ptr, int elem_bytes, uint64_t inner, uint64_t outer, uint64_t ld,
                    uint32_t box_inner, uint32_t box_outer);
int sk_make_tmap_3d(CUtensorMap* out, const void* ptr, uint64_t inner, uint64_t rows, uint64_t batch, uint64_t row_stride,
                    uint64_t batch_stride, uint32_t box_rows);
int sk_pick_bn(int M, int N, int force_bn);
size_t sk_gemm_ws_min_bytes(void);
struct SkGemmEx {
  int M, N, K;
  int batch;
  int a_mode;
  int passes;
  const void *A, *A_lo;
  int lda, a_mn;
  long a_inner, a_rows, a_row_stride, a_batch_stride;
  const void *B, *B_lo;
  int ldb, b_mn;
  void *C, *C_lo;
  int ldc, out_f32;
  const void* bias;
  int bias_f32;
  const void *residual, *residual_lo;
  int ldr, round_before_res, act;
  int col_gin, col_gout;
  int force_bn;
  void* splitk_ws;
  size_t splitk_ws_bytes;
  int pdl;
  int epi;
  const void* aux;
  int ld_aux;
  void* aux_out;
  int ld_aux_out;
  const void *rope_cos, *rope_sin;
  const int* rope_pos;
  int rope_T, rope_cols, rope_maxpos;
};
int sk_gemm_ex_launch(const SkGemmEx& g, cudaStream_t stream);
struct SkGemmPlan;
int sk_gemm_plan_ex(const SkGemmEx& g, SkGemmPlan* out);
int sk_gemm_launch(int M, int N, int K, const void* A, int lda, int a_mn, const void* B, int ldb, int b_mn, void* C,
                   int ldc, int out_f32, const void* bias, const void* residual, int ldr, int round_before_res, int act,
                   int force_bn, cudaStream_t stream, void* splitk_ws = nullptr, size_t splitk_ws_bytes = 0);
SkGemmEx sk_gemm_desc(int M, int N, int K, const void* A, int lda, int a_mn, const void* B, int ldb, int b_mn, void* C,
                      int ldc, int out_f32, const void* bias, const void* residual, int ldr, int round_before_res, int act,
                      int force_bn, void* splitk_ws, size_t splitk_ws_bytes);
int sk_linear_swiglu_fwd_launch(int M, int F, int K, const void* x, const void* Wgu, void* gu, void* act, cudaStream_t s);
int sk_linear_swiglu_bwd_launch(int M, int N, int F, const void* dy, const void* Wd, const void* gu, void* dgu, cudaStream_t s);
int sk_linear_rope_launch(int M, int N, int K, const void* x, const void* W, const void* bias, void* out, const void* cos_t,
                          const void* sin_t, const int32_t* pos_ids, int T, int rope_cols, int max_positions, cudaStream_t s);

int sk_embed_fwd_launch(const int64_t* ids, const bf16* E, bf16* out, int M, int D, int V, cudaStream_t s);
int sk_embed_bwd_launch(const int64_t* ids, const bf16* dx, float* scratch, bf16* dE, int M, int D, int V, int Vpad,
                        int accumulate, cudaStream_t s);
int sk_rmsnorm_fwd_launch(const bf16* x, const bf16* w, bf16* y, float* rstd, int M, int D, float eps, cudaStream_t s);
extern "C" int sk_rmsnorm_bwd_blocks(void);
int sk_rmsnorm_bwd_launch(const bf16* dy, const bf16* x, const bf16* w, const float* rstd, const bf16* dres, bf16* dx,
                          bf16* dw, float* dw_partial, int M, int D, int accumulate_dw, cudaStream_t s);
extern "C" int sk_colsum_splits(void);
int sk_colsum_launch(const bf16* x, bf16* out, float* partial, int M, int N, int ld, int accumulate, cudaStream_t s);
int sk_rope_launch(bf16* qkv, const bf16* cos_t, const bf16* sin_t, const int* pos_ids, int M, int T, int ld,
                   int n_rot_heads, int head_dim, int inverse, int max_positions, cudaStream_t s);
int sk_swiglu_fwd_launch(const bf16* gu, bf16* act, int M, int F, cudaStream_t s);
int sk_swiglu_bwd_launch(const bf16* gu, const bf16* dact, bf16* dgu, int M, int F, cudaStream_t s);
extern "C" int sk_ce_blocks(int M);
int sk_ce_launch(const bf16* logits, const int64_t* labels, bf16* dlogits, float* partial, float* row_nll,
                 float* stats_out, int M, int T, int V, int ldl, float num_items, float dloss, cudaStream_t s,
                 const float* row_weight = nullptr);
int sk_ce_chunk_launch(const bf16* logits_chunk, const int64_t* labels, bf16* dlogits_chunk, float* partial, int row0, int rows,
                       int M, int T, int V, int ldl, float grad_scale, cudaStream_t s);
int sk_ce_finalize_launch(const float* partial, int M, float num_items, float* stats_out, cudaStream_t s);
int sk_gradnorm_launch(const bf16* g, const long* chunk_start, const int* chunk_len, int n_chunks,
                       const int* tensor_chunk_begin, int n_tensors, float* partial, float max_norm, int emulate_bf16,
                       float* stats_out, cudaStream_t s);
int sk_adamw_launch(bf16* p, const bf16* g, bf16* m, bf16* v, long n, float lr, float beta1, float beta2, float eps,
                    float wd, int step, const float* clip_stats, cudaStream_t s);
int sk_transpose_launch(const bf16* in, bf16* out, int M, int N, cudaStream_t s);
int sk_seg_bounds_launch(const int32_t* pos_ids, int32_t* seg_start, int32_t* seg_end, int B, int T, cudaStream_t s);
int sk_layernorm_fwd_launch(const bf16* x, const bf16* w, const bf16* b, bf16* y, float* mean, float* rstd, int M, int D,
                            float eps, cudaStream_t s);
extern "C" int sk_layernorm_bwd_blocks(void);
int sk_layernorm_bwd_launch(const bf16* dy, const bf16* x, const bf16* w, const float* mean, const float* rstd, const bf16* dres,
                            bf16* dx, bf16* dw, bf16* db, float* dw_partial, float* db_partial, int M, int D, int accumulate,
                            cudaStream_t s);
int sk_opt_embed_fwd_launch(const int64_t* ids, const int32_t* pos_ids, const bf16* E, const bf16* P, bf16* out, int M, int T, int D,
                            int V, int n_pos, cudaStream_t s);
int sk_opt_pos_bwd_launch(const int32_t* pos_ids, const bf16* dx, float* scratch, bf16* dP, int M, int T, int D, int n_pos,
                          int accumulate, cudaStream_t s);
int sk_relu_bwd_launch(bf16* g, const bf16* a, long n, cudaStream_t s);

int sk_attn_fwd_launch(const bf16* q, const bf16* k, const bf16* v, bf16* o, float* lse, int B, int T, int H, int KVH,
                       int ld, int ldo, int causal, float scale, cudaStream_t s, const int* seg_start = nullptr);
int sk_attn_bwd_launch(const bf16* q, const bf16* k, const bf16* v, const bf16* o, const bf16* d_o, const float* lse,
                       float* delta, bf16* dq, bf16* dk, bf16* dv, int B, int T, int H, int KVH, int ld, int ldo,
                       int ldg, int causal, float scale, cudaStream_t s, const int* seg_start = nullptr);
int sk_attn_fwd_split_launch(const bf16* q_hi, const bf16* q_lo, const bf16* k_hi, const bf16* k_lo, const bf16* v_hi,
                             const bf16* v_lo, bf16* o_hi, bf16* o_lo, int B, int T, int H, int ld, int ldo, float scale,
                             cudaStream_t s);

int sk_attn_tc_fwd_split_launch(const bf16* qkv_hi, const bf16* qkv_lo, bf16* o_hi, bf16* o_lo, int B, int T, int H, int ld,
                                int ldo, float scale, cudaStream_t s);
int sk_attn_tc_bwd_launch(const bf16* qkv, const bf16* o, const bf16* d_o, const float* lse, float* delta, float* partial,
                          bf16* dqkv, int B, int T, int H, int KVH, int ld, int ldo, int ldg, int causal, float scale,
                          cudaStream_t s, const int* seg_start = nullptr, const int* seg_end = nullptr,
                          const bf16* rope_cos = nullptr, const bf16* rope_sin = nullptr, const int* pos_ids = nullptr,
                          int max_pos = 0);
int sk_attn_tc_fwd_launch(const bf16* qkv, bf16* o, float* lse, int B, int T, int H, int KVH, int ld, int ldo, int causal,
                          float scale, cudaStream_t s, const int* seg_start = nullptr);

int sk_kv_prefill_launch(const bf16* qkv, long layer_stride, int ldq, bf16* cache, const int32_t* lens, int L, int B, int T,
                         int H, int KVH, int T_cache, cudaStream_t s);
int sk_kv_append_launch(const bf16* qkv, int ldq, bf16* kc, bf16* vc, const int32_t* pos, int32_t* lens, int B, int H,
                        int KVH, int T_cache, cudaStream_t s);
int sk_gather_last_launch(const bf16* x, const int32_t* lens, bf16* out, int B, int T, int D, cudaStream_t s);
int sk_attn_decode_splits(int T_cache);
int sk_attn_decode_launch(const bf16* q, int ldq, const bf16* kc, const bf16* vc, const int32_t* lens, bf16* o, int ldo,
                          float* partial, int B, int H, int KVH, int T_cache, float scale, cudaStream_t s);
struct SkSampling;
struct SkDecodeState;
int sk_select_next_launch(const bf16* logits, int ldl, int V, int B, const uint32_t* ban, const SkSampling& cfg,
                          const float* uniforms, const SkDecodeState& st, cudaStream_t s);

int sk_split_f32_launch(const float* x, bf16* hi, bf16* lo, long n, cudaStream_t s);
extern "C" int sk_conv0_nstat(void);
int sk_conv0_launch(const float* wav, const float* w, const float* gamma, const float* beta, double* stats,
                    float2* affine, bf16* out_hi, bf16* out_lo, int B, int S, int pad, int T0, int C, int KW, int ST,
                    float eps, cudaStream_t s);
int sk_layernorm_hilo_launch(const bf16* a_hi, const bf16* a_lo, const bf16* b_hi, const bf16* b_lo, const float* gamma,
                             const float* beta, bf16* o_hi, bf16* o_lo, float* o_f32, int M, int D, float eps,
                             cudaStream_t s);
int sk_regroup_pad_launch(const bf16* in_hi, const bf16* in_lo, bf16* out_hi, bf16* out_lo, int B, int T, int halo,
                          int G, int cg, int cgp, cudaStream_t s);
int sk_row_sqnorm_launch(const float* c, float* out, int U, int D, cudaStream_t s);
int sk_kmeans_argmin_launch(const float* dot, const float* csq, int32_t* labels, int M, int U, int ld, cudaStream_t s);
int sk_rle_launch(const int32_t* labels, const int32_t* n_frames, int32_t* units, int32_t* durations, int32_t* counts,
                  int B, int T, cudaStream_t s);
int sk_rel_len_launch(const int64_t* lens, int32_t* n_frames, int B, int S, int T, cudaStream_t s);
int sk_hilo_to_f32_launch(const bf16* hi, const bf16* lo, float* out, long n, cudaStream_t s);

size_t sk_p2p_flag_bytes_impl();
int sk_p2p_set_trace_impl(void* buf);
int sk_p2p_hog_launch(int ctas, long long ns, unsigned* started, cudaStream_t s);
int sk_p2p_alloc_impl(size_t bytes, void** out);
int sk_p2p_free_impl(void* p);
int sk_p2p_export_impl(const void* ptr, void* handle64, size_t* offset);
int sk_p2p_open_impl(const void* handle64, void** base);
int sk_p2p_close_impl(void* base);
int sk_p2p_signal_launch(void* const* flags, int rank, int world, int slot, uint32_t epoch, cudaStream_t s);
int sk_p2p_wait_launch(void* const* flags, int rank, int world, int slot_lo, int n_slots, uint32_t epoch, int* err_flag, cudaStream_t s);
int sk_p2p_allreduce_launch(void* const* bufs, void* const* flags, int rank, int world, size_t offset_elems, size_t n_elems,
                            int slot, uint32_t epoch, int ctas, int* err_flag, cudaStream_t s);
```

Before: 148,200.

## Add 192/224-wide GEMM tiles and carry-based stream-K for column-unit multiwave

```diff
diff --git a/slamkit_b200/csrc/common.cuh b/slamkit_b200/csrc/common.cuh
--- a/slamkit_b200/csrc/common.cuh
+++ b/slamkit_b200/csrc/common.cuh
@@ -260,9 +260,27 @@
       : "+f"(d[0]), "+f"(d[1]), "+f"(d[2]), "+f"(d[3]), "+f"(d[4]), "+f"(d[5]), "+f"(d[6]), "+f"(d[7]), "+f"(d[8]), "+f"(d[9]), "+f"(d[10]), "+f"(d[11]), "+f"(d[12]), "+f"(d[13]), "+f"(d[14]), "+f"(d[15]), "+f"(d[16]), "+f"(d[17]), "+f"(d[18]), "+f"(d[19]), "+f"(d[20]), "+f"(d[21]), "+f"(d[22]), "+f"(d[23]), "+f"(d[24]), "+f"(d[25]), "+f"(d[26]), "+f"(d[27]), "+f"(d[28]), "+f"(d[29]), "+f"(d[30]), "+f"(d[31]), "+f"(d[32]), "+f"(d[33]), "+f"(d[34]), "+f"(d[35]), "+f"(d[36]), "+f"(d[37]), "+f"(d[38]), "+f"(d[39]), "+f"(d[40]), "+f"(d[41]), "+f"(d[42]), "+f"(d[43]), "+f"(d[44]), "+f"(d[45]), "+f"(d[46]), "+f"(d[47]), "+f"(d[48]), "+f"(d[49]), "+f"(d[50]), "+f"(d[51]), "+f"(d[52]), "+f"(d[53]), "+f"(d[54]), "+f"(d[55]), "+f"(d[56]), "+f"(d[57]), "+f"(d[58]), "+f"(d[59]), "+f"(d[60]), "+f"(d[61]), "+f"(d[62]), "+f"(d[63]), "+f"(d[64]), "+f"(d[65]), "+f"(d[66]), "+f"(d[67]), "+f"(d[68]), "+f"(d[69]), "+f"(d[70]), "+f"(d[71]), "+f"(d[72]), "+f"(d[73]), "+f"(d[74]), "+f"(d[75]), "+f"(d[76]), "+f"(d[77]), "+f"(d[78]), "+f"(d[79]), "+f"(d[80]), "+f"(d[81]), "+f"(d[82]), "+f"(d[83]), "+f"(d[84]), "+f"(d[85]), "+f"(d[86]), "+f"(d[87]), "+f"(d[88]), "+f"(d[89]), "+f"(d[90]), "+f"(d[91]), "+f"(d[92]), "+f"(d[93]), "+f"(d[94]), "+f"(d[95]), "+f"(d[96]), "+f"(d[97]), "+f"(d[98]), "+f"(d[99]), "+f"(d[100]), "+f"(d[101]), "+f"(d[102]), "+f"(d[103]), "+f"(d[104]), "+f"(d[105]), "+f"(d[106]), "+f"(d[107]), "+f"(d[108]), "+f"(d[109]), "+f"(d[110]), "+f"(d[111]), "+f"(d[112]), "+f"(d[113]), "+f"(d[114]), "+f"(d[115]), "+f"(d[116]), "+f"(d[117]), "+f"(d[118]), "+f"(d[119]), "+f"(d[120]), "+f"(d[121]), "+f"(d[122]), "+f"(d[123]), "+f"(d[124]), "+f"(d[125]), "+f"(d[126]), "+f"(d[127])
       : "l"(da), "l"(db), "n"(TA), "n"(TB));
 }
+template <int TA, int TB>
+SK_DEVINL void wgmma_m64n192(float (&d)[96], uint64_t da, uint64_t db) {
+  asm volatile(
+      "{\n\t.reg .pred p;\n\tsetp.eq.u32 p, 1, 1;\n\t"
+      "wgmma.mma_async.sync.aligned.m64n192k16.f32.bf16.bf16 {%0,%1,%2,%3,%4,%5,%6,%7,%8,%9,%10,%11,%12,%13,%14,%15,%16,%17,%18,%19,%20,%21,%22,%23,%24,%25,%26,%27,%28,%29,%30,%31,%32,%33,%34,%35,%36,%37,%38,%39,%40,%41,%42,%43,%44,%45,%46,%47,%48,%49,%50,%51,%52,%53,%54,%55,%56,%57,%58,%59,%60,%61,%62,%63,%64,%65,%66,%67,%68,%69,%70,%71,%72,%73,%74,%75,%76,%77,%78,%79,%80,%81,%82,%83,%84,%85,%86,%87,%88,%89,%90,%91,%92,%93,%94,%95}, %96, %97, p, 1, 1, %98, %99;\n\t}\n"
+      : "+f"(d[0]), "+f"(d[1]), "+f"(d[2]), "+f"(d[3]), "+f"(d[4]), "+f"(d[5]), "+f"(d[6]), "+f"(d[7]), "+f"(d[8]), "+f"(d[9]), "+f"(d[10]), "+f"(d[11]), "+f"(d[12]), "+f"(d[13]), "+f"(d[14]), "+f"(d[15]), "+f"(d[16]), "+f"(d[17]), "+f"(d[18]), "+f"(d[19]), "+f"(d[20]), "+f"(d[21]), "+f"(d[22]), "+f"(d[23]), "+f"(d[24]), "+f"(d[25]), "+f"(d[26]), "+f"(d[27]), "+f"(d[28]), "+f"(d[29]), "+f"(d[30]), "+f"(d[31]), "+f"(d[32]), "+f"(d[33]), "+f"(d[34]), "+f"(d[35]), "+f"(d[36]), "+f"(d[37]), "+f"(d[38]), "+f"(d[39]), "+f"(d[40]), "+f"(d[41]), "+f"(d[42]), "+f"(d[43]), "+f"(d[44]), "+f"(d[45]), "+f"(d[46]), "+f"(d[47]), "+f"(d[48]), "+f"(d[49]), "+f"(d[50]), "+f"(d[51]), "+f"(d[52]), "+f"(d[53]), "+f"(d[54]), "+f"(d[55]), "+f"(d[56]), "+f"(d[57]), "+f"(d[58]), "+f"(d[59]), "+f"(d[60]), "+f"(d[61]), "+f"(d[62]), "+f"(d[63]), "+f"(d[64]), "+f"(d[65]), "+f"(d[66]), "+f"(d[67]), "+f"(d[68]), "+f"(d[69]), "+f"(d[70]), "+f"(d[71]), "+f"(d[72]), "+f"(d[73]), "+f"(d[74]), "+f"(d[75]), "+f"(d[76]), "+f"(d[77]), "+f"(d[78]), "+f"(d[79]), "+f"(d[80]), "+f"(d[81]), "+f"(d[82]), "+f"(d[83]), "+f"(d[84]), "+f"(d[85]), "+f"(d[86]), "+f"(d[87]), "+f"(d[88]), "+f"(d[89]), "+f"(d[90]), "+f"(d[91]), "+f"(d[92]), "+f"(d[93]), "+f"(d[94]), "+f"(d[95])
+      : "l"(da), "l"(db), "n"(TA), "n"(TB));
+}
+template <int TA, int TB>
+SK_DEVINL void wgmma_m64n224(float (&d)[112], uint64_t da, uint64_t db) {
+  asm volatile(
+      "{\n\t.reg .pred p;\n\tsetp.eq.u32 p, 1, 1;\n\t"
+      "wgmma.mma_async.sync.aligned.m64n224k16.f32.bf16.bf16 {%0,%1,%2,%3,%4,%5,%6,%7,%8,%9,%10,%11,%12,%13,%14,%15,%16,%17,%18,%19,%20,%21,%22,%23,%24,%25,%26,%27,%28,%29,%30,%31,%32,%33,%34,%35,%36,%37,%38,%39,%40,%41,%42,%43,%44,%45,%46,%47,%48,%49,%50,%51,%52,%53,%54,%55,%56,%57,%58,%59,%60,%61,%62,%63,%64,%65,%66,%67,%68,%69,%70,%71,%72,%73,%74,%75,%76,%77,%78,%79,%80,%81,%82,%83,%84,%85,%86,%87,%88,%89,%90,%91,%92,%93,%94,%95,%96,%97,%98,%99,%100,%101,%102,%103,%104,%105,%106,%107,%108,%109,%110,%111}, %112, %113, p, 1, 1, %114, %115;\n\t}\n"
+      : "+f"(d[0]), "+f"(d[1]), "+f"(d[2]), "+f"(d[3]), "+f"(d[4]), "+f"(d[5]), "+f"(d[6]), "+f"(d[7]), "+f"(d[8]), "+f"(d[9]), "+f"(d[10]), "+f"(d[11]), "+f"(d[12]), "+f"(d[13]), "+f"(d[14]), "+f"(d[15]), "+f"(d[16]), "+f"(d[17]), "+f"(d[18]), "+f"(d[19]), "+f"(d[20]), "+f"(d[21]), "+f"(d[22]), "+f"(d[23]), "+f"(d[24]), "+f"(d[25]), "+f"(d[26]), "+f"(d[27]), "+f"(d[28]), "+f"(d[29]), "+f"(d[30]), "+f"(d[31]), "+f"(d[32]), "+f"(d[33]), "+f"(d[34]), "+f"(d[35]), "+f"(d[36]), "+f"(d[37]), "+f"(d[38]), "+f"(d[39]), "+f"(d[40]), "+f"(d[41]), "+f"(d[42]), "+f"(d[43]), "+f"(d[44]), "+f"(d[45]), "+f"(d[46]), "+f"(d[47]), "+f"(d[48]), "+f"(d[49]), "+f"(d[50]), "+f"(d[51]), "+f"(d[52]), "+f"(d[53]), "+f"(d[54]), "+f"(d[55]), "+f"(d[56]), "+f"(d[57]), "+f"(d[58]), "+f"(d[59]), "+f"(d[60]), "+f"(d[61]), "+f"(d[62]), "+f"(d[63]), "+f"(d[64]), "+f"(d[65]), "+f"(d[66]), "+f"(d[67]), "+f"(d[68]), "+f"(d[69]), "+f"(d[70]), "+f"(d[71]), "+f"(d[72]), "+f"(d[73]), "+f"(d[74]), "+f"(d[75]), "+f"(d[76]), "+f"(d[77]), "+f"(d[78]), "+f"(d[79]), "+f"(d[80]), "+f"(d[81]), "+f"(d[82]), "+f"(d[83]), "+f"(d[84]), "+f"(d[85]), "+f"(d[86]), "+f"(d[87]), "+f"(d[88]), "+f"(d[89]), "+f"(d[90]), "+f"(d[91]), "+f"(d[92]), "+f"(d[93]), "+f"(d[94]), "+f"(d[95]), "+f"(d[96]), "+f"(d[97]), "+f"(d[98]), "+f"(d[99]), "+f"(d[100]), "+f"(d[101]), "+f"(d[102]), "+f"(d[103]), "+f"(d[104]), "+f"(d[105]), "+f"(d[106]), "+f"(d[107]), "+f"(d[108]), "+f"(d[109]), "+f"(d[110]), "+f"(d[111])
+      : "l"(da), "l"(db), "n"(TA), "n"(TB));
+}
 template <int N, int TA, int TB>
 SK_DEVINL void wgmma_bf16(float (&d)[N / 2], uint64_t da, uint64_t db) {
   if constexpr (N == 256) wgmma_m64n256<TA, TB>(d, da, db);
+  else if constexpr (N == 224) wgmma_m64n224<TA, TB>(d, da, db);
+  else if constexpr (N == 192) wgmma_m64n192<TA, TB>(d, da, db);
   else if constexpr (N == 128) wgmma_m64n128<TA, TB>(d, da, db);
   else wgmma_m64n64<TA, TB>(d, da, db);
 }
diff --git a/slamkit_b200/csrc/gemm_tcgen05.cu b/slamkit_b200/csrc/gemm_tcgen05.cu
--- a/slamkit_b200/csrc/gemm_tcgen05.cu
+++ b/slamkit_b200/csrc/gemm_tcgen05.cu
@@ -2,6 +2,7 @@
 #include <cudaTypedefs.h>
 #include <stdio.h>
 #include <mutex>
+#include <type_traits>
 #include <string.h>
 #include <stdlib.h>
 #include "kernels.h"
@@ -41,6 +42,7 @@
   int sk_groups;
   int sk_G;
   int sk_colunits;
+  int sk_carry;
   int units, n_groups;
   float* sk_ws;
   uint32_t* sk_flags;
@@ -63,6 +65,7 @@
   static constexpr int STAGING_BYTES = 4 * 2 * 4096;
   static constexpr int BAR_BYTES = 256;
   static constexpr int SMEM_BYTES = STAGES * STAGE_BYTES + STAGING_BYTES + BAR_BYTES + 1024;
+  static_assert(BN % 64 == 0 || (BN == 224 && EW == 4), "a 32-column tail chunk only on the 224-wide tile");
   static_assert(STAGES * STAGE_BYTES >= BM * BN * 4, "the parked fp32 accumulator must fit in the stage ring");
   static_assert(SMEM_BYTES <= 227 * 1024, "sm_90 allows 227 KB of shared memory per block");
 };
@@ -93,6 +96,11 @@
     asm volatile("ld.shared.v4.b32 {%0, %1, %2, %3}, [%4];"
                  : "=r"(r[4 * i]), "=r"(r[4 * i + 1]), "=r"(r[4 * i + 2]), "=r"(r[4 * i + 3])
                  : "r"(acc_chunk_addr<BN>(base, row, c0 + i)) : "memory");
+}
+
+SK_DEVINL uint32_t staging_addr(uint32_t sbuf, int lane, int j, bool tail) {
+  return tail ? sbuf + (uint32_t)lane * 64u + (uint32_t)((j ^ ((lane >> 1) & 3)) << 4)
+              : sbuf + (uint32_t)lane * 128u + (uint32_t)((j ^ (lane & 7)) << 4);
 }
 
 SK_DEVINL float gelu_erf(float y) {
@@ -110,7 +118,7 @@
 template <bool SK>
 struct WorkIter {
   int num_kb, splits, kb_per_split, total_items, tiles_n;
-  int G, colunits, units, n_groups, sk_groups, grp, mem;
+  int G, colunits, carry, units, n_groups, sk_groups, grp, mem;
   long sk_total, sk_cur, sk_end;
   int next_unit, next_item;
   int tile, split, kb_begin, kb_end, role;
@@ -123,6 +131,7 @@
     tiles_n = p.tiles_n;
     G = p.sk_G;
     colunits = p.sk_colunits;
+    carry = p.sk_carry;
     units = p.units;
     n_groups = p.n_groups;
     sk_groups = p.sk_groups;
@@ -146,6 +155,19 @@
   }
   SK_DEVINL int tile_of(int unit) const { return colunits ? mem * tiles_n + unit : unit * G + mem; }
   SK_DEVINL bool next() {
+    if (SK && sk_cur < sk_end && carry) {
+      const int unit = (int)((sk_end - 1) / num_kb);
+      const long ustart = (long)unit * num_kb;
+      const long b = sk_cur > ustart ? sk_cur : ustart;
+      kb_begin = (int)(b - ustart);
+      kb_end = (int)(sk_end - ustart);
+      unit_end_it = ustart + num_kb;
+      tile = tile_of(unit);
+      split = 0;
+      role = kb_begin != 0 ? 3 : (kb_end < num_kb ? 1 : 0);
+      sk_end = b;
+      return true;
+    }
     if (SK && sk_cur < sk_end) {
       const int unit = (int)(sk_cur / num_kb);
       kb_begin = (int)(sk_cur - (long)unit * num_kb);
@@ -276,6 +298,8 @@
   using Cfg = GemmCfg<BN, EW>;
   static_assert(EW == 4 || (EW == 8 && BN == 256 && !SK), "8 epilogue warps: plain 256-wide tiles only");
   constexpr int CS = EW / 4;
+  constexpr int NC64 = BN / 64;
+  constexpr bool TAIL = BN % 64 != 0;
   griddep_launch();
   extern __shared__ uint8_t smem_raw[];
   const uint32_t smem_base = (smem_u32(smem_raw) + 1023u) & ~1023u;
@@ -381,6 +405,34 @@
         float acc[BN / 2];
 #pragma unroll
         for (int i = 0; i < BN / 2; ++i) acc[i] = 0.f;
+        if (SK && w.role == 3) {
+          const int src = (int)blockIdx.x - w.G;
+          if (threadIdx.x == 0) {
+            for (int qq = 0; qq < 4; ++qq) {
+              const uint32_t* f = p.sk_flags + src * 4 + qq;
+              const uint64_t t0 = globaltimer_ns();
+              while (ld_acquire_u32(f) == 0u) {
+                __nanosleep(64);
+                if (globaltimer_ns() - t0 > 8000000000ull) __trap();
+              }
+            }
+            for (int qq = 0; qq < 4; ++qq) p.sk_flags[src * 4 + qq] = 0u;
+          }
+          named_bar_sync(1, 256);
+          const float* slot = p.sk_ws + (size_t)src * SK_SLOT_FLOATS;
+          const int r0 = 64 * wg + 16 * (warp & 3) + (lane >> 2);
+#pragma unroll
+          for (int j = 0; j < BN / 8; ++j) {
+            const int col = 8 * j + 2 * (lane & 3);
+#pragma unroll
+            for (int h = 0; h < 2; ++h) {
+              const float2 v = __ldcg(reinterpret_cast<const float2*>(slot + sk_slot_off(col >> 5, (col & 31) >> 2, r0 + 8 * h) +
+                                                                      (col & 3)));
+              acc[4 * j + 2 * h] = v.x;
+              acc[4 * j + 2 * h + 1] = v.y;
+            }
+          }
+        }
         const int k_iters = max(0, w.kb_end - w.kb_begin);
         int prev = -1;
         for (int kb = 0; kb < k_iters; ++kb) {
@@ -541,26 +593,31 @@
           }
           __syncwarp();
         }
-        auto stage_store = [&](const CUtensorMap* map, const uint32_t (&pk)[32], int col) {
+        auto stage_store = [&](const CUtensorMap* map, const uint32_t (&pk)[32], int col, auto tail_c) {
+          constexpr bool tail = decltype(tail_c)::value;
           const uint32_t sbuf = staging_base + (EW == 4 ? (uint32_t)warp * 8192u + (store_cnt & 1u) * 4096u : (uint32_t)warp * 4096u);
           if (lane == 0) {
             if constexpr (EW == 4) tma_store_wait_read<1>(); else tma_store_wait_read<0>();
           }
           __syncwarp();
 #pragma unroll
-          for (int j = 0; j < 8; ++j) {
-            const uint32_t dst = sbuf + (uint32_t)lane * 128u + (uint32_t)((j ^ (lane & 7)) << 4);
-            asm volatile("st.shared.v4.b32 [%0], {%1, %2, %3, %4};" ::"r"(dst), "r"(pk[4 * j]), "r"(pk[4 * j + 1]),
-                         "r"(pk[4 * j + 2]), "r"(pk[4 * j + 3])
+          for (int j = 0; j < (tail ? 4 : 8); ++j) {
+            asm volatile("st.shared.v4.b32 [%0], {%1, %2, %3, %4};" ::"r"(staging_addr(sbuf, lane, j, tail)), "r"(pk[4 * j]),
+                         "r"(pk[4 * j + 1]), "r"(pk[4 * j + 2]), "r"(pk[4 * j + 3])
                          : "memory");
           }
           fence_proxy_async();
           __syncwarp();
           if (lane == 0) {
-            tma_store_2d(map, sbuf, col, m0 + q * 32);
+            tma_store_2d(tail ? &tmAux : map, sbuf, col, m0 + q * 32);
             tma_store_commit();
           }
           ++store_cnt;
+        };
+        auto for_chunks = [&](auto&& body) {
+#pragma unroll 1
+          for (int c2 = chalf * (NC64 / CS); c2 < (chalf + 1) * (NC64 / CS); ++c2) body(std::false_type{}, c2);
+          if constexpr (TAIL) body(std::true_type{}, NC64);
         };
         if (!SK && p.tma_store && p.epi == 1) {
           if constexpr (BN == 256) {
@@ -578,7 +635,7 @@
                   gpk[16 + t] = pack_bf16(__uint_as_float(r1[2 * t]), __uint_as_float(r1[2 * t + 1]));
                 }
               }
-              stage_store(&tmC, gpk, n0 + i * 64);
+              stage_store(&tmC, gpk, n0 + i * 64, std::false_type{});
               {
                 uint32_t r0[32], r1[32];
                 acc_ld(taddr + 128 + i * 64, r0);
@@ -589,14 +646,14 @@
                   upk[16 + t] = pack_bf16(__uint_as_float(r1[2 * t]), __uint_as_float(r1[2 * t + 1]));
                 }
               }
-              stage_store(&tmC, upk, n0 + 128 + i * 64);
+              stage_store(&tmC, upk, n0 + 128 + i * 64, std::false_type{});
 #pragma unroll
               for (int t = 0; t < 32; ++t) {
                 const float2 gf = unpack_bf16(gpk[t]), uf = unpack_bf16(upk[t]);
                 const float2 sb = unpack_bf16(pack_bf16(silu_f(gf.x), silu_f(gf.y)));
                 gpk[t] = pack_bf16(sb.x * uf.x, sb.y * uf.y);
               }
-              stage_store(&tmAux, gpk, (n0 >> 1) + i * 64);
+              stage_store(&tmAux, gpk, (n0 >> 1) + i * 64, std::false_type{});
             }
           }
         } else if (!SK && p.tma_store && p.epi == 3) {
@@ -656,48 +713,48 @@
                 pk[16 + g * 4 + e] = pack_bf16(v1[2 * e], v1[2 * e + 1]);
               }
             }
-            stage_store(&tmC, pk, col64);
+            stage_store(&tmC, pk, col64, std::false_type{});
           }
         } else if (p.tma_store && !p.bias && !p.residual && !p.act) {
-#pragma unroll 1
-          for (int c2 = chalf * (BN / 64 / CS); c2 < (chalf + 1) * (BN / 64 / CS); ++c2) {
+          for_chunks([&](auto tail_c, int c2) {
+            constexpr bool tail = decltype(tail_c)::value;
             uint32_t r0[32], r1[32], pk[32];
             acc_ld(taddr + c2 * 64, r0);
-            acc_ld(taddr + c2 * 64 + 32, r1);
-            if (SK && n_contrib > 0) {
-              sk_fixup_add(r0, p.sk_ws, c2 * 2, row_in_tile, first_contrib, w.G, n_contrib);
-              sk_fixup_add(r1, p.sk_ws, c2 * 2 + 1, row_in_tile, first_contrib, w.G, n_contrib);
-            }
-#pragma unroll
-            for (int t = 0; t < 16; ++t) {
-              pk[t] = pack_bf16(__uint_as_float(r0[2 * t]), __uint_as_float(r0[2 * t + 1]));
-              pk[16 + t] = pack_bf16(__uint_as_float(r1[2 * t]), __uint_as_float(r1[2 * t + 1]));
-            }
-            stage_store(&tmC, pk, n0 + c2 * 64);
-          }
+            if (SK && n_contrib > 0) sk_fixup_add(r0, p.sk_ws, c2 * 2, row_in_tile, first_contrib, w.G, n_contrib);
+#pragma unroll
+            for (int t = 0; t < 16; ++t) pk[t] = pack_bf16(__uint_as_float(r0[2 * t]), __uint_as_float(r0[2 * t + 1]));
+            if constexpr (!tail) {
+              acc_ld(taddr + c2 * 64 + 32, r1);
+              if (SK && n_contrib > 0) sk_fixup_add(r1, p.sk_ws, c2 * 2 + 1, row_in_tile, first_contrib, w.G, n_contrib);
+#pragma unroll
+              for (int t = 0; t < 16; ++t) pk[16 + t] = pack_bf16(__uint_as_float(r1[2 * t]), __uint_as_float(r1[2 * t + 1]));
+            }
+            stage_store(&tmC, pk, n0 + c2 * 64, tail_c);
+          });
         } else if (p.tma_store && !p.bias && !p.act && p.residual && !p.residual_lo) {
-#pragma unroll 1
-          for (int c2 = chalf * (BN / 64 / CS); c2 < (chalf + 1) * (BN / 64 / CS); ++c2) {
+          for_chunks([&](auto tail_c, int c2) {
+            constexpr bool tail = decltype(tail_c)::value;
+            constexpr int nj = tail ? 4 : 8;
             const int col64 = n0 + c2 * 64;
-            if (col64 >= p.N) break;
+            if (col64 >= p.N) return;
             uint4 rv[8];
             if (row_ok) {
               const bf16* rp = p.residual + row * p.ldr + col64;
 #pragma unroll
-              for (int j = 0; j < 8; ++j) rv[j] = (col64 + 8 * j < p.N) ? ldg128(rp + 8 * j) : make_uint4(0u, 0u, 0u, 0u);
+              for (int j = 0; j < 8; ++j) rv[j] = (j < nj && col64 + 8 * j < p.N) ? ldg128(rp + 8 * j) : make_uint4(0u, 0u, 0u, 0u);
             } else {
 #pragma unroll
               for (int j = 0; j < 8; ++j) rv[j] = make_uint4(0u, 0u, 0u, 0u);
             }
             uint32_t r0[32], r1[32], pk[32];
             acc_ld(taddr + c2 * 64, r0);
-            acc_ld(taddr + c2 * 64 + 32, r1);
-            if (SK && n_contrib > 0) {
-              sk_fixup_add(r0, p.sk_ws, c2 * 2, row_in_tile, first_contrib, w.G, n_contrib);
-              sk_fixup_add(r1, p.sk_ws, c2 * 2 + 1, row_in_tile, first_contrib, w.G, n_contrib);
-            }
-#pragma unroll
-            for (int j = 0; j < 8; ++j) {
+            if (SK && n_contrib > 0) sk_fixup_add(r0, p.sk_ws, c2 * 2, row_in_tile, first_contrib, w.G, n_contrib);
+            if constexpr (!tail) {
+              acc_ld(taddr + c2 * 64 + 32, r1);
+              if (SK && n_contrib > 0) sk_fixup_add(r1, p.sk_ws, c2 * 2 + 1, row_in_tile, first_contrib, w.G, n_contrib);
+            }
+#pragma unroll
+            for (int j = 0; j < nj; ++j) {
               const uint32_t* r = j < 4 ? r0 + 8 * j : r1 + 8 * (j - 4);
               const uint32_t rw[4] = {rv[j].x, rv[j].y, rv[j].z, rv[j].w};
 #pragma unroll
@@ -711,18 +768,18 @@
                 pk[4 * j + e] = pack_bf16(a0 + f.x, a1 + f.y);
               }
             }
-            stage_store(&tmC, pk, col64);
-          }
+            stage_store(&tmC, pk, col64, tail_c);
+          });
         } else if (p.tma_store) {
-#pragma unroll 1
-          for (int c2 = chalf * (BN / 64 / CS); c2 < (chalf + 1) * (BN / 64 / CS); ++c2) {
+          for_chunks([&](auto tail_c, int c2) {
+            constexpr bool tail = decltype(tail_c)::value;
             const uint32_t sbuf = staging_base + (EW == 4 ? (uint32_t)warp * 8192u + (store_cnt & 1u) * 4096u : (uint32_t)warp * 4096u);
             if (lane == 0) {
               if constexpr (EW == 4) tma_store_wait_read<1>(); else tma_store_wait_read<0>();
             }
             __syncwarp();
 #pragma unroll
-            for (int half = 0; half < 2; ++half) {
+            for (int half = 0; half < (tail ? 1 : 2); ++half) {
               uint32_t r[32];
               acc_ld(taddr + c2 * 64 + half * 32, r);
               if (SK && n_contrib > 0) sk_fixup_add(r, p.sk_ws, c2 * 2 + half, row_in_tile, first_contrib, w.G, n_contrib);
@@ -736,21 +793,20 @@
                   epi_bias_act(v, p, col);
                   if (row_ok) epi_residual(v, p, row, col);
                 }
-                const int j = half * 4 + g;
-                const uint32_t dst = sbuf + (uint32_t)lane * 128u + (uint32_t)((j ^ (lane & 7)) << 4);
-                asm volatile("st.shared.v4.b32 [%0], {%1, %2, %3, %4};" ::"r"(dst), "r"(pack_bf16(v[0], v[1])),
-                             "r"(pack_bf16(v[2], v[3])), "r"(pack_bf16(v[4], v[5])), "r"(pack_bf16(v[6], v[7]))
+                asm volatile("st.shared.v4.b32 [%0], {%1, %2, %3, %4};" ::"r"(staging_addr(sbuf, lane, half * 4 + g, tail)),
+                             "r"(pack_bf16(v[0], v[1])), "r"(pack_bf16(v[2], v[3])), "r"(pack_bf16(v[4], v[5])),
+                             "r"(pack_bf16(v[6], v[7]))
                              : "memory");
               }
             }
             fence_proxy_async();
             __syncwarp();
             if (lane == 0) {
-              tma_store_2d(&tmC, sbuf, n0 + c2 * 64, m0 + q * 32);
+              tma_store_2d(tail ? &tmAux : &tmC, sbuf, n0 + c2 * 64, m0 + q * 32);
               tma_store_commit();
             }
             ++store_cnt;
-          }
+          });
         }
         else
 #pragma unroll 1
@@ -868,14 +924,15 @@
   SK_REQUIRE((reinterpret_cast<uintptr_t>(ptr) & 15) == 0, "TMA base pointer must be 16-byte aligned");
   SK_REQUIRE((ld * elem_bytes) % 16 == 0, "TMA row pitch must be a multiple of 16 bytes (ld=%llu)",
              (unsigned long long)ld);
-  SK_REQUIRE(box_inner * elem_bytes == 128, "SW128 box inner extent must be 128 bytes");
+  SK_REQUIRE(box_inner * elem_bytes == 128 || box_inner * elem_bytes == 64, "box inner extent must be 128 (or 64) bytes");
   cuuint64_t dims[2] = {inner, outer};
   cuuint64_t strides[1] = {ld * (uint64_t)elem_bytes};
   cuuint32_t box[2] = {box_inner, box_outer};
   cuuint32_t estr[2] = {1, 1};
   CUtensorMapDataType dt = elem_bytes == 2 ? CU_TENSOR_MAP_DATA_TYPE_BFLOAT16 : CU_TENSOR_MAP_DATA_TYPE_FLOAT32;
   CUresult r = g_encode(out, dt, 2, const_cast<void*>(ptr), dims, strides, box, estr, CU_TENSOR_MAP_INTERLEAVE_NONE,
-                        CU_TENSOR_MAP_SWIZZLE_128B, CU_TENSOR_MAP_L2_PROMOTION_L2_256B,
+                        box_inner * elem_bytes == 64 ? CU_TENSOR_MAP_SWIZZLE_64B : CU_TENSOR_MAP_SWIZZLE_128B,
+                        CU_TENSOR_MAP_L2_PROMOTION_L2_256B,
                         CU_TENSOR_MAP_FLOAT_OOB_FILL_NONE);
   SK_REQUIRE(r == CUDA_SUCCESS, "cuTensorMapEncodeTiled failed with CUresult %d (inner=%llu outer=%llu ld=%llu)", (int)r,
              (unsigned long long)inner, (unsigned long long)outer, (unsigned long long)ld);
@@ -927,7 +984,7 @@
   return launch_gemm<BN, true, true, SK, EW>(tm, p, grid, s);
 }
 
-inline int tile_cost(int bn) { return bn >= 256 ? 100 : (bn >= 128 ? 61 : 54); }
+inline int tile_cost(int bn) { return bn >= 256 ? 100 : (bn > 128 ? 61 + (bn - 128) * 39 / 128 : (bn == 128 ? 61 : 54)); }
 
 constexpr size_t SK_FLAG_BYTES = 4096;
 
@@ -935,20 +992,28 @@
 
 size_t sk_gemm_ws_min_bytes(void) { return (size_t)sk_num_sms() * SK_SLOT_FLOATS * sizeof(float) + SK_FLAG_BYTES; }
 
-int sk_pick_bn(int M, int N, int force_bn) {
+int sk_pick_bn(int M, int N, int force_bn, bool fit_forced, bool fit, bool whole_heads) {
   if (force_bn == 64 || force_bn == 128 || force_bn == 256) return force_bn;
+  if (fit_forced && (force_bn == 192 || (force_bn == 224 && !whole_heads))) return force_bn;
   const int nsm = sk_num_sms();
-  const int cands[3] = {256, 128, 64};
+  auto cost = [&](int bn) {
+    const long tiles = (long)((M + BM - 1) / BM) * ((N + bn - 1) / bn);
+    return ((tiles + nsm - 1) / nsm) * tile_cost(bn);
+  };
   int best = 256;
-  long best_cost = -1;
-  for (int i = 0; i < 3; ++i) {
-    const int bn = cands[i];
-    const long tiles = (long)((M + BM - 1) / BM) * ((N + bn - 1) / bn);
-    const long waves = (tiles + nsm - 1) / nsm;
-    const long cost = waves * tile_cost(bn);
-    if (best_cost < 0 || cost * 100 < best_cost * 75) {
-      best_cost = cost;
+  long best_cost = cost(256);
+  for (const int bn : {128, 64}) {
+    if (cost(bn) * 100 < best_cost * 75) {
+      best_cost = cost(bn);
       best = bn;
+    }
+  }
+  if (best == 256 && fit && N % 256 != 0) {
+    for (const int bn : {224, 192}) {
+      if (!(whole_heads && bn % 64 != 0) && cost(bn) * 100 < best_cost * 95) {
+        best_cost = cost(bn);
+        best = bn;
+      }
     }
   }
   return best;
@@ -986,7 +1051,12 @@
   const bool sk_ok = sk_env != 0 && g.batch == 1 && !use3d && g.passes == 1 && g.a_mode == 0 && g.splitk_ws != nullptr &&
                      g.splitk_ws_bytes >= sk_gemm_ws_min_bytes();
   const size_t ws_data_bytes = g.splitk_ws_bytes > SK_FLAG_BYTES ? g.splitk_ws_bytes - SK_FLAG_BYTES : 0;
-  BN = (g.a_mode == 1) ? 64 : sk_pick_bn(g.M * g.batch, g.N, (g.epi == 1 || g.epi == 2) ? 256 : g.force_bn);
+  const bool fit = g.passes == 1 && g.batch == 1 && !use3d && g.a_mode == 0 && g.epi != 1 && g.epi != 2;
+  SK_REQUIRE((g.force_bn != 192 && g.force_bn != 224) || (fit && !(g.force_bn == 224 && g.epi == 3)),
+             "gemm: force_bn=%d needs a one-pass 2-D problem (and whole 64-column heads for RoPE)", g.force_bn);
+  BN = (g.a_mode == 1) ? 64
+                       : sk_pick_bn(g.M * g.batch, g.N, (g.epi == 1 || g.epi == 2) ? 256 : g.force_bn, fit,
+                                    fit && !sk_ok, g.epi == 3);
   memset(&p, 0, sizeof(p));
   p.M = g.M; p.N = g.N; p.K = g.K;
   p.batch = g.batch;
@@ -1052,16 +1122,24 @@
     }
   }
   p.sk_G = 1;
-  if (sk_ok && BN == 256 && p.splits == 1 && num_kb >= sk_min_kb && (p.tiles_n <= 8 || (sk_env >= 2 && p.tiles_m <= 8))) {
+  if (sk_ok && BN == 256 && p.splits == 1 && num_kb >= sk_min_kb && (p.tiles_n <= 8 || p.tiles_m <= 8)) {
     const int colunits = p.tiles_n <= 8 ? 0 : 1;
     const int G = colunits ? p.tiles_m : p.tiles_n;
     const int units = colunits ? p.tiles_n : p.tiles_m;
     const int n_groups = nsm / G;
     const int rem = units % n_groups;
     const long slots = ((long)(units + n_groups - 1) / n_groups) * n_groups;
-    if (n_groups >= 1 && rem != 0 && (slots - units) * 100 >= slots * sk_min_idle) {
-      p.sk_units = rem;
-      p.sk_groups = n_groups < rem * sk_ranges ? n_groups : rem * sk_ranges;
+    const bool multiwave = units > n_groups;
+    if (n_groups >= 1 && rem != 0 && (slots - units) * 100 >= slots * sk_min_idle &&
+        (!colunits || multiwave || sk_env >= 2)) {
+      if (colunits && multiwave) {
+        p.sk_units = rem + n_groups;
+        p.sk_groups = n_groups;
+        p.sk_carry = 1;
+      } else {
+        p.sk_units = rem;
+        p.sk_groups = n_groups < rem * sk_ranges ? n_groups : rem * sk_ranges;
+      }
       p.sk_G = G;
       p.sk_colunits = colunits;
       p.units = units;
@@ -1131,6 +1209,9 @@
   if (g.epi == 1) {
     const int rc3 = sk_make_tmap_2d(&tm[5], g.aux_out, 2, (uint64_t)g.N / 2, (uint64_t)g.M, (uint64_t)g.ld_aux_out, 64, 32);
     if (rc3) return rc3;
+  } else if (p.tma_store && BN % 64 != 0) {
+    const int rc3 = sk_make_tmap_2d(&tm[5], g.C, 2, (uint64_t)g.N, (uint64_t)g.M, (uint64_t)g.ldc, 32, 32);
+    if (rc3) return rc3;
   }
   int rc;
   if (p.sk_units > 0) {
@@ -1140,6 +1221,8 @@
   } else {
     switch (BN) {
       case 256: rc = dispatch_major<256, false>(g.a_mn, g.b_mn, tm, p, grid, stream); break;
+      case 224: rc = dispatch_major<224, false>(g.a_mn, g.b_mn, tm, p, grid, stream); break;
+      case 192: rc = dispatch_major<192, false>(g.a_mn, g.b_mn, tm, p, grid, stream); break;
       case 128: rc = dispatch_major<128, false>(g.a_mn, g.b_mn, tm, p, grid, stream); break;
       default:  rc = dispatch_major<64, false>(g.a_mn, g.b_mn, tm, p, grid, stream); break;
     }
diff --git a/slamkit_b200/csrc/kernels.h b/slamkit_b200/csrc/kernels.h
--- a/slamkit_b200/csrc/kernels.h
+++ b/slamkit_b200/csrc/kernels.h
@@ -5,7 +5,7 @@
                     uint32_t box_inner, uint32_t box_outer);
 int sk_make_tmap_3d(CUtensorMap* out, const void* ptr, uint64_t inner, uint64_t rows, uint64_t batch, uint64_t row_stride,
                     uint64_t batch_stride, uint32_t box_rows);
-int sk_pick_bn(int M, int N, int force_bn);
+int sk_pick_bn(int M, int N, int force_bn, bool fit_forced, bool fit, bool whole_heads);
 size_t sk_gemm_ws_min_bytes(void);
 struct SkGemmEx {
   int M, N, K;
```

Measured after the change: 153,100 (median of 6 runs). 1.03x the previous value.
